# pathint/RankCompV3.jl

Hardware: AMD Instinct MI355X
Metric: gene-pair·sample comparisons/sec at 20k genes × 1k samples (higher is better)
Workload: dtype u16

## Files before the change

### rankcompv3.jl_amd/_ffi.py

```python
from __future__ import annotations

import ctypes
import os
import subprocess
from typing import NamedTuple

import numpy as np

_HERE = os.path.dirname(os.path.abspath(__file__))
LIB_PATH = os.environ.get("REO_LIB_PATH") or os.path.join(_HERE, "libreo_hip.so")
CSRC = os.path.join(_HERE, "csrc")

REO_OK, REO_EINVAL, REO_EHIP, REO_ECOMM, REO_ENOMEM = 0, -1, -2, -3, -4
NTIMINGS = 12
CALL_BINS = 8192

SYMBOLS = [
    "reo_version", "reo_last_error", "reo_create", "reo_destroy", "reo_trim_memory", "reo_set_shard", "reo_set_allreduce", "reo_set_allgather",
    "reo_create_multi", "reo_comm_unique_id", "reo_comm_init_rank",
    "reo_set_matrix_f64", "reo_set_matrix_i64", "reo_set_matrix_dev_f64", "reo_set_matrix_dev_i64",
    "reo_set_matrix_f32", "reo_set_matrix_i32", "reo_set_matrix_dev_f32", "reo_set_matrix_dev_i32",
    "reo_set_matrix_rm_f64", "reo_set_matrix_rm_i64", "reo_set_matrix_rm_f32", "reo_set_matrix_rm_i32",
    "reo_set_matrix_csc_f64", "reo_set_matrix_csc_i64", "reo_set_matrix_csc_f32", "reo_set_matrix_csc_i32",
    "reo_set_groups", "reo_compute_thresholds", "reo_set_thresholds", "reo_get_thresholds", "reo_threshold",
# ... 649 lines not shown
        pm = self._partner_mask(partner_mask)
        n_sel = np.zeros(g.size, dtype=np.int32)
        n_gt = np.zeros((g.size, max(self.S, 1)), dtype=np.int32)
        n_eq = np.zeros_like(n_gt) if ties else None
        self.sample_counts_raw(g, mask, pm, n_sel, n_gt, n_eq)
        return SampleCounts(g, n_sel, n_gt[:, : self.S], None if n_eq is None else n_eq[:, : self.S])

    def sample_scores(self, genes, partner_mask=None) -> SampleScores:
        return sample_scores_from(self.sample_counts(genes, "n13", partner_mask), self.sample_counts(genes, "n31", partner_mask))

    def sample_tests_raw(self, genes, partner_mask, n_above_ctrl, n_below_ctrl, rev_up, rev_down, tied, p_up, p_down) -> None:
        check(self._L.reo_sample_tests(self._h, *_genes(genes), _opt(partner_mask), _opt(n_above_ctrl), _opt(n_below_ctrl), _opt(rev_up),
                                       _opt(rev_down), _opt(tied), _opt(p_up), _opt(p_down)))

    def sample_tests(self, genes=None, partner_mask=None, counts=True) -> SampleTests:
        g = np.arange(self.G, dtype=np.int32) if genes is None else np.ascontiguousarray(genes, dtype=np.int32).reshape(-1)
        pm = self._partner_mask(partner_mask)
        shape = (g.size, max(self.S, 1))
        n_above, n_below = np.zeros(g.size, dtype=np.int32), np.zeros(g.size, dtype=np.int32)
        ints = [np.zeros(shape, dtype=np.int32) for _ in range(3)] if counts else [None] * 3
        p_up, p_down = np.ones(shape, dtype=np.float64), np.ones(shape, dtype=np.float64)
        self.sample_tests_raw(g, pm, n_above, n_below, ints[0], ints[1], ints[2], p_up, p_down)
        cut = lambda a: None if a is None else a[:, : self.S]
        return SampleTests(g, n_above, n_below, cut(ints[0]), cut(ints[1]), cut(ints[2]), cut(p_up), cut(p_down))

    def sample_calls_raw(self, genes, partner_mask, pval_deg: float, padj_deg: float, calls, cut, n_up, n_down) -> None:
        check(self._L.reo_sample_calls(self._h, *_genes(genes), _opt(partner_mask), float(pval_deg), float(padj_deg), _opt(calls), _opt(cut),
                                       _opt(n_up), _opt(n_down)))

    def sample_calls(self, pval_deg: float, padj_deg: float, genes=None, partner_mask=None) -> SampleCalls:
        g = np.arange(self.G, dtype=np.int32) if genes is None else np.ascontiguousarray(genes, dtype=np.int32).reshape(-1)
        pm = self._partner_mask(partner_mask)
        S = max(self.S, 1)
        calls = np.zeros((g.size, S), dtype=np.int8)
        cut, n_up, n_down = (np.zeros(S, dtype=np.int32) for _ in range(3))
        self.sample_calls_raw(g, pm, pval_deg, padj_deg, calls, cut, n_up, n_down)
        return SampleCalls(g, calls[:, : self.S], cut[: self.S], n_up[: self.S], n_down[: self.S])

    def pair_support_raw(self, genes, rowptr, partner, n_gt, n_eq, outcome) -> None:
        check(self._L.reo_pair_support(self._h, *_genes(genes), _opt(rowptr), _genes(partner)[0],
                                       _opt(n_gt), _opt(n_eq), _opt(outcome)))

    def pair_support(self, pairs, ties=True, outcomes=False) -> PairSupport:
        code = None
        if isinstance(pairs, PairList):
            genes, rowptr, partner, code = pairs
        else:
            genes, rowptr, partner = pairs
        g = np.ascontiguousarray(genes, dtype=np.int32).reshape(-1)
        rp = np.ascontiguousarray(rowptr, dtype=np.int64).reshape(-1)
        pa = np.ascontiguousarray(partner, dtype=np.int32).reshape(-1)
        if rp.size != g.size + 1:
            raise DimensionMismatch(REO_EINVAL, f"pair_support: rowptr has {rp.size} entries for {g.size} rows (one more is needed)")
        if rp.size and int(rp[-1]) != pa.size:
            raise DimensionMismatch(REO_EINVAL, f"pair_support: rowptr lists {int(rp[-1])} entries, partner has {pa.size}")
        if code is not None:
            code = np.asarray(code)
            if code.size != pa.size:
                raise DimensionMismatch(REO_EINVAL, f"pair_support: code has {code.size} entries, partner has {pa.size}")
        n, ng, S = pa.size, max(self.ngroups, 1), max(self.S, 1)
        n_gt = np.zeros((n, ng), dtype=np.int32)
        n_eq = np.zeros_like(n_gt) if ties else None
        outcome = np.zeros((n, S), dtype=np.uint8) if outcomes else None
        if g.size:
            self.pair_support_raw(g, rp, pa, n_gt, n_eq, outcome)
        sizes = np.bincount(np.asarray(self._group_id, dtype=np.int64), minlength=ng)[:ng].astype(np.int64)
        return PairSupport(g, rp, pa, code, n_gt, n_eq, None if outcome is None else outcome[:, : self.S], sizes)

    def mccullagh(self, cont) -> np.ndarray:
        cont = np.ascontiguousarray(cont, dtype=np.int32).reshape(-1, 9)
        out = np.zeros((cont.shape[0], 5), dtype=np.float64)
        check(self._L.reo_mccullagh(self._h, _ptr(cont), cont.shape[0], _ptr(out)))
        return out

    @staticmethod
    def _pseudobulk_args(cells, order, chunk_ptr):
        order = np.ascontiguousarray(order, dtype=np.int32)
        chunk_ptr = np.ascontiguousarray(chunk_ptr, dtype=np.int32)
        n_out = chunk_ptr.size - 1
        if hasattr(cells, "tocsc"):
            m = cells.tocsc()
            m.sort_indices()
            G, C = m.shape
            isint = np.issubdtype(m.dtype, np.integer)
            val = np.ascontiguousarray(m.data, dtype=np.int64 if isint else np.float64)
            colptr = np.ascontiguousarray(m.indptr, dtype=np.int64)
            rowidx = np.ascontiguousarray(m.indices, dtype=np.int32)
            args = (G, C, _ptr(colptr), _ptr(rowidx), _ptr(val), _ptr(order), order.size, _ptr(chunk_ptr), n_out)
            return "csc", "i64" if isint else "f64", args, G, (m, val, colptr, rowidx, order, chunk_ptr)
        X = np.asarray(cells)
        isint = np.issubdtype(X.dtype, np.integer)
        Xf = np.asfortranarray(X, dtype=np.int64 if isint else np.float64)
        G, C = Xf.shape
        args = (_ptr(Xf), G, C, G, _ptr(order), order.size, _ptr(chunk_ptr), n_out)
        return "dense", "i64" if isint else "f64", args, G, (Xf, order, chunk_ptr)

    def pseudobulk(self, cells, order, chunk_ptr) -> np.ndarray:
        form, ty, args, G, keep = self._pseudobulk_args(cells, order, chunk_ptr)
        out = np.zeros((G, args[-1]), dtype=np.int64 if ty == "i64" else np.float64, order="F")
        check(getattr(self._L, f"reo_pseudobulk_{form}_{ty}")(self._h, *args, _ptr(out)))
        return out

    def set_matrix_pseudobulk(self, cells, order, chunk_ptr) -> None:
        if is_device_sparse(cells) or is_device_tensor(cells):
            order = np.ascontiguousarray(order, dtype=np.int32)
            chunk_ptr = np.ascontiguousarray(chunk_ptr, dtype=np.int32)
            n_out = chunk_ptr.size - 1
            tail = (_ptr(order) if order.size else None, order.size, _ptr(chunk_ptr), n_out)
            if is_device_sparse(cells):
                ty, G, C, nnz, colptr, rowidx, val, bits, keep = device_csc_entry(cells)
                check(getattr(self._L, "reo_set_matrix_pseudobulk_csc_dev_" + ty)(self._h, G, C, nnz, _dptr(colptr), _dptr(rowidx), bits, _dptr(val), *tail))
            else:
                ptr, G, C, ld, ty, keep = device_matrix(cells)
                check(getattr(self._L, "reo_set_matrix_pseudobulk_dense_dev_" + ty)(self._h, ctypes.c_void_p(ptr), G, C, ld, *tail))
            self.G, self.S = G, n_out
            return
        form, ty, args, G, keep = self._pseudobulk_args(cells, order, chunk_ptr)
        check(getattr(self._L, f"reo_set_matrix_pseudobulk_{form}_{ty}")(self._h, *args))
        self.G, self.S = G, args[-1]

    def filter_matrix(self, min_profiles: int = 0, min_features: int = 0):
        info = self.info()
        pk = np.zeros(info["S"], dtype=np.uint8)
        gk = np.zeros(info["G"], dtype=np.uint8)
        sk, gkn = ctypes.c_int64(0), ctypes.c_int64(0)
        check(self._L.reo_filter_matrix(self._h, int(min_profiles), int(min_features), _ptr(pk) if pk.size else None, _ptr(gk) if gk.size else None,
                                        ctypes.byref(sk), ctypes.byref(gkn)))
        self.G, self.S = int(gkn.value), int(sk.value)
        return pk.astype(bool), gk.astype(bool)

    def get_matrix(self) -> np.ndarray:
        info = self.info()
        dt = {1: np.float64, 2: np.int64, 3: np.float32}.get(info["resident_dtype"])
        if dt is None:
            raise DimensionMismatch(REO_EINVAL, "no expression matrix set")
        out = np.zeros((info["G"], info["S"]), dtype=dt, order="F")
        check(self._L.reo_get_matrix(self._h, _ptr(out), out.nbytes))
        return out

    def set_profiling(self, on: bool) -> None:
        check(self._L.reo_set_profiling(self._h, 1 if on else 0))

    def reset_timings(self) -> None:
        check(self._L.reo_reset_timings(self._h))

    def timings(self) -> dict:
        ms = np.zeros(NTIMINGS, dtype=np.float64)
        check(self._L.reo_get_timings(self._h, _ptr(ms), NTIMINGS))
        return {"transform_ms": ms[0], "k1_ms": ms[1], "k2_ms": ms[2], "iter_ms": ms[3], "k3_ms": max(ms[3] - ms[2], 0.0), "k2_launches": int(ms[4]),
                "k1_launches": int(ms[5]), "exchange_ms": ms[6], "pseudobulk_ms": ms[7], "k2_full_ms": ms[8],
                "k2_full_launches": int(ms[9]), "k2_delta_ms": ms[10], "set_matrix_host_wall_ms": ms[11]}

    def info(self) -> dict:
        w = np.zeros(30, dtype=np.int64)
        check(self._L.reo_get_info(self._h, _ptr(w), 30))
        v = np.zeros(28, dtype=np.int64)
        v[:] = w[:28]
        return {"G": int(v[0]), "S": int(v[1]), "Gp": int(v[2]), "table_bytes": int(v[3]), "has_ties": int(v[4]),
                "tiles_owned": int(v[5]), "tiles_total": int(v[6]), "tile_i": int(v[7]), "chunk_j": int(v[8]),
                "chunks_per_panel": int(v[9]), "unit_h": int(v[10]), "sample_slots": int(v[11]),
                "shared_group_counts": int(v[12]), "group_count_bytes": int(v[13]), "transform_in_lds": int(v[14]), "xcc_local_histograms": int(v[15]),
                "cycle_period": int(v[16]), "cycle_found_at_pass": int(v[17]), "cycle_passes_skipped": int(v[18]), "upload_link_bytes": int(v[19]),
                "eager_range_launches": int(v[20]), "rowmajor_upload": int(v[21]),
                "csc_upload": int(v[22]), "csc_nnz": int(v[23]), "resident_dtype": int(v[24]),
                "k1_slot_order": int(v[25]), "k1_half_tiles_separated": int(v[26]), "csc_device": int(v[27]),
                "k1_unslot_form": int(w[28]), "contrast_treat": int(w[29])}
```

### rankcompv3.jl_amd/csrc/api.hip

```cpp
#include <execinfo.h>
#include <signal.h>
#include <unistd.h>

#include <ctime>
#include <algorithm>
#include <chrono>
#include <cmath>
#include <cstdarg>
#include <cstdio>
#include <cstdlib>
#include <cstring>

#include "reo_internal.h"
#include "contrast.h"
#include "upload_csc.h"

#include <mutex>
#include <unordered_map>

namespace reo {

static thread_local std::string g_err;
thread_local bool tl_release_synced = false;

// ... 157 lines not shown
void tic(reo_ctx *c, int slot)
{
    if (!c->profiling) return;
    StageTimer t;
    if (!c->pool.empty()) { t = c->pool.back(); c->pool.pop_back(); }
    else { (void)handle_event(&t.a, 1); (void)handle_event(&t.b, 1); }
    (void)hipEventRecord(t.a, c->stream);
    c->pending.emplace_back(slot, t);
    c->open.push_back(c->pending.size() - 1);
}

void toc(reo_ctx *c)
{
    if (!c->profiling || c->open.empty()) return;
    (void)hipEventRecord(c->pending[c->open.back()].second.b, c->stream);
    c->open.pop_back();
}

void collect_timings(reo_ctx *c)
{
    for (auto &pr : c->pending) {
        float ms = 0.f;
        (void)hipEventSynchronize(pr.second.b);
        if (hipEventElapsedTime(&ms, pr.second.a, pr.second.b) == hipSuccess) {
            c->t_ms[pr.first] += ms;
            if (pr.first == 2 && !c->k2_modes.empty()) {
                if (c->k2_seen < c->k2_modes.size()) {
                    if (c->k2_modes[c->k2_seen]) { c->t_ms[8] += ms; c->t_ms[9] += 1.0; }
                    else c->t_ms[10] += ms;
                }
                ++c->k2_seen;
            }
        }
        c->pool.push_back(pr.second);
    }
    c->pending.clear();
    c->open.clear();
    c->k2_modes.clear();
    c->k2_seen = 0;
}

static int32_t major_reo_lower_count(int32_t n, double thr)
{
    const long double ln2 = 0.693147180559945309417232121458L;
    long double logc = 0.0L, cdf_prev = 0.0L;
    int32_t first_above = -1;
    double pmin = 1.0;
    for (int x = 0; x <= n / 2; ++x) {
        if (x > 0) logc += std::log(static_cast<long double>(n - x + 1)) - std::log(static_cast<long double>(x));
        long double cdf = x >= n ? 1.0L : cdf_prev + std::exp(logc - static_cast<long double>(n) * ln2);
        if (cdf > 1.0L) cdf = 1.0L;
        const long double hi = 1.0L - cdf_prev;
        long double p = 2.0L * (cdf < hi ? cdf : hi);
        if (p > 1.0L) p = 1.0L;
        if (x == 0) {
            pmin = static_cast<double>(p);
            if (!(pmin < thr)) return n;
        }
        if (static_cast<double>(p) > thr) { first_above = x; break; }
        cdf_prev = cdf;
    }
    return first_above < 0 ? -1 : n - first_above + 1;
}

static hipError_t stream_wait(reo_ctx *c)
{
    if (!c->spin_wait) return hipStreamSynchronize(c->stream);
    for (unsigned spin = 0;; ++spin) {
        const hipError_t q = hipStreamQuery(c->stream);
        if (q != hipErrorNotReady) return q;
        if (spin > (1u << 22)) return hipStreamSynchronize(c->stream);
    }
}

static struct sigaction g_old_action[3];

static void segv_backtrace(int sig)
{
    static const char head[] = "libreo_hip: fatal signal, native backtrace of the faulting thread:\n";
    (void)!write(2, head, sizeof head - 1);
    void *frames[64];
    const int n = backtrace(frames, 64);
    backtrace_symbols_fd(frames, n, 2);
    sigaction(sig, &g_old_action[sig == SIGSEGV ? 0 : (sig == SIGBUS ? 1 : 2)], nullptr);
    raise(sig);
}

static void install_segv_backtrace()
{
    static bool done = false;
    if (done) return;
    done = true;
    void *warm[2];
    (void)backtrace(warm, 2);
    struct sigaction sa;
    memset(&sa, 0, sizeof sa);
    sa.sa_handler = segv_backtrace;
    sa.sa_flags = SA_NODEFER;
    sigaction(SIGSEGV, &sa, &g_old_action[0]);
    sigaction(SIGBUS, &sa, &g_old_action[1]);
    sigaction(SIGABRT, &sa, &g_old_action[2]);
}

static double wall_us()
{
    timespec ts;
    clock_gettime(CLOCK_MONOTONIC, &ts);
    return ts.tv_sec * 1e6 + ts.tv_nsec * 1e-3;
}

static void drop_ref_mask(reo_ctx *c, const char *why)
{
    c->ref_slot = -1;
    c->ref_gone = why;
}

int32_t wait_or_drop_table(reo_ctx *c)
{
    const hipError_t e = stream_wait(c);
    if (e == hipSuccess) return REO_OK;
    c->built_k = -1;
    c->table_complete = false;
    drop_ref_mask(c, "a kernel queued on this context failed and the class table was dropped");
    set_error("a kernel queued on this context failed: %s (the class table was dropped: call reo_build_pairs again)", hipGetErrorString(e));
    return REO_EHIP;
}

int32_t use(reo_ctx *c)
{
    if (!c) { set_error("null context"); return REO_EINVAL; }
    REO_HIP_CHECK(hipSetDevice(c->device));
    return REO_OK;
}

int32_t no_multi(reo_ctx *c, const char *what)
{
    if (!c) { set_error("null context"); return REO_EINVAL; }
    if (c->in_multi) {
        set_error("%s is not available on a reo_create_multi context (every device would need the matrix: use one process per GPU, each with its own context)", what);
        return REO_EINVAL;
    }
    return REO_OK;
}

static void invalidate(reo_ctx *c)
{
    drop_ref_mask(c, "the matrix or the groups changed after the last reo_identify_degs (reo_set_matrix_*, reo_filter_matrix, reo_set_groups): "
                     "the class table it ran on is gone");
    c->transformed = false;
    c->built_k = -1;
    c->built_treat = -1;
    c->gc_valid = false;
    c->eager_k1 = false;
    c->last_k1_slots = 0; c->k1_slot_items = nullptr; c->k1_slot_items_n = 0; c->k1_slot_gp = 0;
}

static size_t elem_bytes(int dtype) { return dtype >= 3 ? 4 : 8; }

static int32_t check_shape(int64_t G, int64_t S)
{
    if (G < 2 || G > kMaxGenes || S < 2 || S > (1 << 20)) {
        set_error("matrix is %lld x %lld; G must be in [2, %d] and S in [2, 1048576]", (long long)G, (long long)S, kMaxGenes);
        return REO_EINVAL;
    }
    return REO_OK;
}

static int32_t set_matrix(reo_ctx *c, const void *X, int64_t G, int64_t S, int64_t ld, int dtype, bool on_device, int layout = kLayoutColMajor)
{
    const bool rowmajor = layout == kLayoutRowMajor;
    int32_t rc = use(c);
    if (rc) return rc;
    if (dtype >= 3 && getenv("REO_TRANSFORM") && getenv("REO_TRANSFORM")[0] == 's') {
        set_error("REO_TRANSFORM=segmented: the segmented sort of the A/B build takes Float64 and Int64 matrices only, not Float32 / Int32");
        return REO_EINVAL;
    }
    if (!X) { set_error("matrix pointer is null"); return REO_EINVAL; }
    if ((rc = check_shape(G, S))) return rc;
    if (rowmajor && ld < S) { set_error("row pitch %lld < S = %lld (row-major: ld counts the elements from one gene's row to the next)", (long long)ld, (long long)S); return REO_EINVAL; }
    if (layout == kLayoutColMajor && ld < G) { set_error("leading dimension %lld < G = %lld", (long long)ld, (long long)G); return REO_EINVAL; }
    invalidate(c);
    c->rowmajor_upload = 0;
    c->csc_upload = 0; c->csc_nnz = 0; c->csc_device = 0;
    const bool host_i32 = dtype == 4 && !on_device;
    const size_t resident = static_cast<size_t>(G) * S * (dtype == 3 ? 4 : 8);
    c->G = G; c->S = S; c->dtype = dtype == 4 ? 2 : dtype;
    if (on_device && dtype == 4) {
        if ((rc = c->dX_owned.ensure(resident))) return rc;
        c->dX = c->dX_owned.p; c->ld = G;
        if ((rc = widen_device_i32(c, X, ld, G, S, c->dX_owned.p))) { invalidate(c); c->dtype = 0; return rc; }
        if (hipStreamSynchronize(c->stream) != hipSuccess) { set_error("widening the Int32 matrix failed"); invalidate(c); c->dtype = 0; return REO_EHIP; }
    } else if (on_device) {
        c->dX = X; c->ld = ld;
        c->dX_owned.release();
    } else {
        if ((rc = c->dX_owned.ensure(resident))) return rc;
        c->dX = c->dX_owned.p; c->ld = G;
        const bool lds_ranking = G <= 65535 && !(getenv("REO_TRANSFORM") && getenv("REO_TRANSFORM")[0] == 's');
        if (c->eager_mode > 0 && lds_ranking && static_cast<int64_t>(c->group_id.size()) == S && !c->in_multi) {
            const bool k1 = c->eager_mode > 1 && c->ngroups == 2 && c->thr_set && c->world <= 1 && !c->comm && !c->ag && !c->ar && c->k1_wave &&
                            S <= 65535 && !c->k1_stamps;
            c->Gp = static_cast<int>((c->G + kGenePad - 1) / kGenePad) * kGenePad;
            c->Wp = c->Gp / 32;
            if ((rc = c->table.ensure(static_cast<size_t>(c->G) * kPlanes * c->Wp))) return rc;
            const double w0 = wall_us();
            struct DrainUp {
                reo_ctx *c;
                ~DrainUp() { if (c->up) (void)hipStreamSynchronize(c->up); if (c->rk) (void)hipStreamSynchronize(c->rk); }
            } drain_up{c};
            DrainOnExit drain(c);
            rc = eager_upload(c, X, ld, k1, host_i32, layout);
            if (rc) { invalidate(c); return rc; }
            c->rowmajor_upload = rowmajor ? 1 : 0;
            c->csc_upload = layout == kLayoutCsc ? 1 : 0;
            drain.dismiss();
            c->t_ms[11] += (wall_us() - w0) * 1e-3;
            if (c->eager_k1) { c->built_k = 0; c->table_complete = true; }
            return REO_OK;
        }
        struct DrainUp2 {
            reo_ctx *c;
            ~DrainUp2() { if (c->up) (void)hipStreamSynchronize(c->up); }
        } drain_up{c};
        DrainOnExit drain(c);
        const double w0 = wall_us();
        if ((rc = upload_columns(c, X, ld, G, S, c->dX_owned.p, dtype, layout))) { invalidate(c); return rc; }
        c->rowmajor_upload = rowmajor ? 1 : 0;
        c->csc_upload = layout == kLayoutCsc ? 1 : 0;
        drain.dismiss();
        c->t_ms[11] += (wall_us() - w0) * 1e-3;
    }
    return REO_OK;
}

int32_t ensure_transform(reo_ctx *c)
{
    if (c->dtype == 0) { set_error("no expression matrix set"); return REO_EINVAL; }
    if (c->group_id.empty()) { set_error("no groups set"); return REO_EINVAL; }
    if (static_cast<int64_t>(c->group_id.size()) != c->S) {
        set_error("'data' and 'group' do not have compatible sizes (%lld columns, %zu group labels)",
                  (long long)c->S, c->group_id.size());
        return REO_EINVAL;
    }
    if (c->transformed) return REO_OK;
    c->Gp = static_cast<int>((c->G + kGenePad - 1) / kGenePad) * kGenePad;
    c->Wp = c->Gp / 32;
    c->table_prezeroed = false;
    int32_t rc = c->table.ensure(static_cast<size_t>(c->G) * kPlanes * c->Wp);
    if (rc) return rc;
    return run_transform(c);
}

static int32_t ensure_iter_buffers(reo_ctx *c)
{
    int32_t rc;
    const size_t G = c->G;
    for (int t = 0; t < 2; ++t) {
        if ((rc = c->refbits[t].ensure(c->Wp))) return rc;
        if ((rc = c->refbytes[t].ensure(c->Gp))) return rc;
    }
    if ((rc = c->raw.ensure(G * kRaw)) ||
        (rc = c->delta_list.ensure(2 * static_cast<size_t>(c->Gp))) || (rc = c->cont.ensure(G * 9)) || (rc = c->result.ensure(G * 15)) ||
        (rc = c->sorted_d.ensure((G + 63) / 64 * 64 + (G + 63) / 64)) || (rc = c->sorted_p.ensure(G)) || (rc = c->rank_s.ensure(G)) ||
        (rc = c->rank_a.ensure(G)) || (rc = c->scal.ensure(8)) || (rc = c->blockmin.ensure(std::max<size_t>(64, (G + 1023) / 1024))) ||
        (rc = c->state.ensure(1)) ||
        (rc = c->chunk_v.ensure(((G + kSortChunk - 1) / kSortChunk) * (kSortChunk + kSortChunk / 32))) ||
        (rc = c->chunk_i.ensure(((G + kSortChunk - 1) / kSortChunk) * kSortChunk)) || (rc = c->part.ensure(3 * (std::max<size_t>(65536, (G + kSortChunk - 1) / kSortChunk * kSortChunk) / 16 + 8))) ||
        (rc = c->cand.ensure(2 * 1024)) || (rc = c->gridbar.ensure(4)) || (rc = c->hist.ensure(3 * kHistParts * ((G + 32767) / 32768 * 32768))) || (rc = c->olist.ensure(2 * kOneStride)) || (rc = c->mrank.ensure(c->Gp)) || (rc = c->lstate.ensure(1)) || (rc = c->clist.ensure(2 * kListStride)) || (rc = c->scal.ensure(64)))
        return rc;
    if (!c->host_state) REO_HIP_CHECK(pool_alloc(reinterpret_cast<void **>(&c->host_state), sizeof(IterState), true));
    return REO_OK;
}

static int32_t upload_ref(reo_ctx *c, const uint8_t *ref, int slot, int32_t *nref)
{
    int32_t n = 0;
    for (int64_t i = 0; i < c->G; ++i) n += ref[i] != 0;
    *nref = n;
    REO_HIP_CHECK(hipMemsetAsync(c->refbytes[slot].p, 0, c->Gp, c->stream));
    REO_HIP_CHECK(hipMemcpyAsync(c->refbytes[slot].p, ref, c->G, hipMemcpyHostToDevice, c->stream));
    return launch_pack_ref(c, c->refbytes[slot].p, c->refbits[slot].p);
}

static int32_t init_state(reo_ctx *c, int32_t nref)
{
    IterState st;
    memset(&st, 0, sizeof st);
    st.nref = nref;
    st.nref_prev = nref;
    st.delta_cnt[0] = st.delta_cnt[1] = 0x7FFFFFFF;
    st.need_full = 1;
    st.raw_pass = -1;
    st.kstar = -1;
    *c->host_state = st;
    REO_HIP_CHECK(hipMemcpyAsync(c->state.p, c->host_state, sizeof st, hipMemcpyHostToDevice, c->stream));
    return REO_OK;
}

static int32_t exchange_table(reo_ctx *c)
{
    if (c->x_pipelined) {
        c->table_complete = true;
        return REO_OK;
    }
    c->table_complete = c->world <= 1;
    if (c->world <= 1 && !c->comm) return REO_OK;
    int32_t rc;
    if (c->comm || c->ag) {
        const int64_t bytes = exchange_unit_words(c) * exchange_units_per_rank(c) * static_cast<int64_t>(sizeof(uint32_t));
        if ((rc = c->xsend.ensure(static_cast<size_t>(bytes / 4))) || (rc = c->xrecv.ensure(static_cast<size_t>(bytes / 4) * c->world))) return rc;
        tic(c, 6);
        if ((rc = launch_pack_units(c))) return rc;
        if (c->comm) {
            if ((rc = comm_allgather(c, c->xsend.p, c->xrecv.p, bytes)) < 0) return rc;
        } else {
            rc = c->ag(c->xsend.p, c->xrecv.p, bytes, c->stream, c->ag_user);
            if (rc) { set_error("all-gather hook failed with %d", rc); return REO_ECOMM; }
        }
        if ((rc = launch_expand_units(c))) return rc;
        toc(c);
    } else {
        if (!c->ar) return REO_OK;
        const int64_t count = static_cast<int64_t>(c->G) * kPlanes * c->Wp;
        tic(c, 6);
        rc = c->ar(c->table.p, count, c->stream, c->ar_user);
        toc(c);
        if (rc) { set_error("all-reduce hook failed with %d", rc); return REO_ECOMM; }
    }
    c->table_complete = true;
    return REO_OK;
}

static int32_t pass_fault(reo_ctx *c)
{
    const int32_t f = c->host_state ? c->host_state->fault : 0;
    if (!f) return REO_OK;
    if (f == kFaultTallies) {
        set_error("the iteration passes met tallies that no class table can produce (a gene pair in two states at once): the table in "
                  "this context is not what reo_build_pairs makes -- an exchange hook delivered wrong words and the scan of its "
                  "table was switched off (REO_CHECK_HOOK_TABLE=0)");
        c->built_k = -1;
        c->table_complete = false;
    } else {
        set_error("the persistent iteration kernel gave up at a grid barrier (a workgroup did not arrive within its bound); "
                  "REO_LIGHT=1 runs the same passes as separate launches");
    }
    return REO_EHIP;
}

int32_t upload_slot2col(reo_ctx *c, const std::vector<int32_t> &map)
{
    if (map == c->sc_slot2col_host && c->sc_slot2col.p == c->sc_slot2col_uploaded) return REO_OK;
    c->sc_slot2col_host = map;
    c->sc_slot2col_uploaded = nullptr;
    REO_HIP_CHECK(hipMemcpyAsync(c->sc_slot2col.p, c->sc_slot2col_host.data(), map.size() * sizeof(int32_t), hipMemcpyHostToDevice, c->stream));
    c->sc_slot2col_uploaded = c->sc_slot2col.p;
    return REO_OK;
}

int32_t need_complete_table(reo_ctx *c)
{
    if (c->built_k < 0) { set_error("no class table: call reo_build_pairs first"); return REO_EINVAL; }
    if (!c->table_complete) {
        set_error("shard %d of %d holds only its own part of the class table: attach a communicator (reo_comm_init_rank) or an "
                  "exchange hook (reo_set_allgather, reo_set_allreduce) before reo_build_pairs", c->rank, c->world);
        return REO_ECOMM;
    }
    return REO_OK;
}

}

using namespace reo;

extern "C" {

int32_t reo_version(void) { return 1100; }

int32_t reo_trim_memory(void)
{
    std::vector<Block> all;
    {
        Pool &P = pool();
        std::lock_guard<std::mutex> lk(P.mu);
        all.swap(P.free_blocks);
        P.cached = 0;
    }
    int dev = 0;
    const bool have_dev = hipGetDevice(&dev) == hipSuccess;
    for (const Block &b : all) {
        if (!b.pinned) (void)hipSetDevice(b.device);
        raw_free(b.p, b.pinned);
    }
    {
        Handles &H = handles();
        std::lock_guard<std::mutex> lk(H.mu);
        for (int k = 0; k < 2; ++k) {
            for (auto &st : H.streams[k]) { (void)hipSetDevice(st.first); (void)hipStreamDestroy(st.second); }
            for (auto &ev : H.events[k]) { (void)hipSetDevice(ev.first); (void)hipEventDestroy(ev.second); }
            H.streams[k].clear(); H.events[k].clear();
        }
    }
    if (have_dev) (void)hipSetDevice(dev);
    return REO_OK;
}

const char *reo_last_error(void) { return g_err.c_str(); }

int32_t reo_create(reo_ctx **out, int32_t device, uint64_t seed)
{
    if (!out) { set_error("out is null"); return REO_EINVAL; }
    *out = nullptr;
    if (getenv("REO_DEBUG_SEGV")) install_segv_backtrace();
    int ndev = 0;
    if (hipGetDeviceCount(&ndev) != hipSuccess || ndev == 0) {
        set_error("no HIP device visible: libreo_hip has no CPU fallback");
        return REO_EHIP;
    }
    if (device < 0) REO_HIP_CHECK(hipGetDevice(&device));
    if (device >= ndev) { set_error("device %d out of range (%d visible)", device, ndev); return REO_EINVAL; }
    hipDeviceProp_t prop;
    REO_HIP_CHECK(hipGetDeviceProperties(&prop, device));
    if (strncmp(prop.gcnArchName, "gfx950", 6) != 0) {
        set_error("device %d is %s; this library carries gfx950 (MI355X) code objects only", device, prop.gcnArchName);
        return REO_EHIP;
    }
    REO_HIP_CHECK(hipSetDevice(device));
    reo_ctx *c = new (std::nothrow) reo_ctx();
    if (!c) { set_error("out of host memory"); return REO_ENOMEM; }
    c->device = device;
    c->seed = seed;
    if (const char *e = getenv("REO_K1_WAVE")) c->k1_wave = (e[0] != '0');
    if (const char *e = getenv("REO_K1_HALF")) c->k1_half = (e[0] != '0');
    if (const char *e = getenv("REO_K1_SLOTS")) c->k1_slots = (e[0] != '0');
    if (const char *e = getenv("REO_K1_QUEUE")) c->k1_queue = (e[0] != '0');
    if (const char *e = getenv("REO_K1_UNSLOT")) { const int v = atoi(e); c->k1_unslot = (v == 8 || v == 4) ? v : (e[0] == '0' ? 0 : -1); }
    if (const char *e = getenv("REO_K1_WORKERS")) c->k1_workers = std::max(1, atoi(e));
    if (const char *e = getenv("REO_K1_ORDER")) c->k1_order = std::max(0, std::min(2, atoi(e)));
    {
        int n = 0;
        if (hipDeviceGetAttribute(&n, hipDeviceAttributeMultiprocessorCount, c->device) == hipSuccess && n > 0) c->n_cus = n;
    }
    if (const char *e = getenv("REO_SPIN_WAIT")) c->spin_wait = (e[0] != '0');
    if (const char *e = getenv("REO_CHECK_HOOK_TABLE")) c->check_hook_table = (e[0] != '0');
    if (const char *e = getenv("REO_SHARE_GROUP_COUNTS")) c->share_counts = (e[0] != '0');
    if (const char *e = getenv("REO_LIGHT_BAND")) c->light_band = std::max(0, atoi(e));
    if (const char *e = getenv("REO_HIST_BELOW")) c->hist_below = std::max(0, atoi(e));
    if (const char *e = getenv("REO_CYCLE")) c->cycle_watch = atoi(e) != 0;
    if (const char *e = getenv("REO_LIGHT")) c->light_mode = e[0] == '0' ? 0 : (e[0] == '2' ? 2 : (e[0] == '3' ? 3 : 1));
    c->light_window = light_window(); c->light_min_g = light_min_genes();
    if (const char *e = getenv("REO_LIGHT_WINDOW")) c->light_window = std::max(1, std::min(31, atoi(e)));
    if (const char *e = getenv("REO_LIGHT_MIN_G")) c->light_min_g = std::max(64, atoi(e));
    if (const char *e = getenv("REO_STATE_MIRROR")) c->state_mirror_wanted = (e[0] != '0');
    if (const char *e = getenv("REO_EXCHANGE_WAVES")) c->x_waves = std::max(1, std::min(8, atoi(e)));
    if (const char *e = getenv("REO_EAGER_UPLOAD")) c->eager_mode = std::max(0, std::min(2, atoi(e)));
    if (const char *e = getenv("REO_EAGER_CHUNK")) c->eager_chunk = std::max(1, atoi(e));
    if (const char *e = getenv("REO_EAGER_GATE")) c->eager_gate = atoi(e) != 0;
    if (const char *e = getenv("REO_EAGER_RANGES")) c->eager_ranges = std::max(1, std::min(6, atoi(e)));
    if (const char *e = getenv("REO_UPLOAD_THREADS")) c->upload_threads = std::max(0, std::min(64, atoi(e)));
    c->debug_passes = getenv("REO_DEBUG_PASSES") != nullptr;
    c->debug_stamps = getenv("REO_DEBUG_STAMPS") != nullptr;
    c->k1_stamps = getenv("REO_K1_STAMPS") != nullptr;
    hipError_t e = handle_stream(&c->stream, 0);
    if (e != hipSuccess) { delete c; set_error("hipStreamCreate failed: %s", hipGetErrorString(e)); return REO_EHIP; }
    int ok = 0;
    const char *xe = getenv("REO_XCC_LOCAL");
    if (!(xe && xe[0] == '0')) {
        const int32_t rc = xcc_selftest(c, &ok);
        if (rc) { reo_destroy(c); return rc; }
    }
    c->xcc_local = ok;
    *out = c;
    return REO_OK;
}

void reo_destroy(reo_ctx *c)
{
    if (!c) return;
    for (reo_ctx *p : c->peers) reo_destroy(p);
    c->peers.clear();
    (void)hipSetDevice(c->device);
    for (int q = 0; q < 2; ++q) if (c->k1s[q]) (void)hipStreamSynchronize(c->k1s[q]);
    if (c->xs) (void)hipStreamSynchronize(c->xs);
    if (c->up) (void)hipStreamSynchronize(c->up);
    if (c->rk) (void)hipStreamSynchronize(c->rk);
    (void)hipStreamSynchronize(c->stream);
    comm_release(c);
    collect_timings(c);
    tl_release_synced = true;
    for (auto &t : c->pool) { release_event(t.a, 1); release_event(t.b, 1); }
    c->dX_owned.release(); c->pos.release(); c->lo.release(); c->hi.release(); c->goff_dev.release();
    c->table.release();
    c->t_kin.release(); c->t_kout.release(); c->t_vin.release(); c->t_vout.release(); c->t_temp.release();
    c->t_order.release(); c->t_flags.release(); c->t_slots.release(); c->unit_map.release();
    for (auto &il : c->k1_wave_items) il.buf.release();
    for (int q = 0; q < 2; ++q) { release_stream(c->k1s[q], 0); release_event(c->ev_k1_join[q], 0); }
    release_stream(c->xs, 0);
    release_stream(c->up, 0);
    release_stream(c->rk, 1);
    for (auto &e : c->ev_rk) release_event(e, 0);
    for (auto &e : c->ev_up) release_event(e, 0);
    c->e_lists.release();
    for (int q = 0; q < 3; ++q) {
        if (c->stage_h[q]) pool_free(c->stage_h[q], c->stage_cap, true);
        c->stage_d[q].release();
        release_event(c->ev_stage[q], 0);
        release_event(c->ev_widen[q], 0);
    }
    release_event(c->ev_fork, 0);
    release_event(c->ev_x, 0);
    for (auto &e : c->ev_k1) release_event(e, 0);
    c->t_pos16.release(); c->t_lo16.release(); c->t_hi16.release(); c->gcounts.release();
    c->k1_slot_part.release(); c->k1_slot_maps.release(); c->pos_s.release(); c->lo_s.release(); c->k1_queue_ctr.release();
    c->t_pos32.release(); c->t_lo32.release(); c->t_hi32.release(); c->t_vin32.release(); c->t_vout32.release();
    for (int t = 0; t < 2; ++t) { c->refbits[t].release(); c->refbytes[t].release(); }
    c->raw.release(); c->delta_list.release(); c->cont.release(); c->result.release(); c->sorted_d.release(); c->sorted_p.release();
    c->rank_s.release(); c->rank_a.release(); c->scal.release(); c->blockmin.release();
    c->state.release(); c->trace.release(); c->modes.release(); c->cand.release(); c->hist.release(); c->mrank.release(); c->lstate.release(); c->clist.release(); c->olist.release(); c->units_all.release(); c->xsend.release(); c->xrecv.release(); c->check_flag.release(); c->gridbar.release(); c->chunk_v.release(); c->chunk_i.release(); c->part.release();
    if (c->host_state) pool_free(c->host_state, sizeof(IterState), true);
    if (c->host_flags) pool_free(c->host_flags, 8 * sizeof(int32_t), true);
    release_event(c->ev_flags, 0);
    if (c->host_ref) pool_free(c->host_ref, c->host_ref_cap, true);
    release_stream(c->stream, 0);
    delete c;
    tl_release_synced = false;
}

int32_t reo_set_shard(reo_ctx *c, int32_t rank, int32_t world)
{
    if (!c) { set_error("null context"); return REO_EINVAL; }
    if (world < 1 || rank < 0 || rank >= world) { set_error("bad shard %d of %d", rank, world); return REO_EINVAL; }
    if (!c->peers.empty()) { set_error("a multi-GPU context (reo_create_multi) shards by itself"); return REO_EINVAL; }
    c->rank = rank; c->world = world;
    c->built_k = -1;
    drop_ref_mask(c, "reo_set_shard dropped the class table that the last reo_identify_degs ran on");
    c->eager_k1 = false;
    c->gc_valid = false;
    c->table_complete = false;
    return REO_OK;
}

int32_t reo_set_allreduce(reo_ctx *c, reo_allreduce_fn fn, void *user)
{
    if (!c) { set_error("null context"); return REO_EINVAL; }
    c->ar = fn; c->ar_user = user;
    return REO_OK;
}

int32_t reo_set_allgather(reo_ctx *c, reo_allgather_fn fn, void *user)
{
    if (!c) { set_error("null context"); return REO_EINVAL; }
    c->ag = fn; c->ag_user = user;
    return REO_OK;
}

static int32_t set_matrix_all(reo_ctx *c, const void *X, int64_t G, int64_t S, int64_t ld, int dtype, bool on_device, int layout = kLayoutColMajor)
{
    int32_t rc = set_matrix(c, X, G, S, ld, dtype, on_device, layout);
    for (size_t d = 0; d < (c ? c->peers.size() : 0) && !rc; ++d) {
        reo_ctx *p = c->peers[d];
        if (!on_device) { rc = set_matrix(p, X, G, S, ld, dtype, false, layout); continue; }
        const void *src = dtype == 4 ? c->dX : X;
        const int64_t sld = dtype == 4 ? G : ld;
        const size_t eb = dtype == 4 ? 8 : elem_bytes(dtype);
        if ((rc = use(p)) || (rc = p->dX_owned.ensure(static_cast<size_t>(G) * S * eb))) break;
        if (hipMemcpy2DAsync(p->dX_owned.p, static_cast<size_t>(G) * eb, src, static_cast<size_t>(sld) * eb, static_cast<size_t>(G) * eb, static_cast<size_t>(S),
                             hipMemcpyDefault, p->stream) != hipSuccess) {
            set_error("peer copy of the matrix to device %d failed", p->device); rc = REO_EHIP;
        }
        if (!rc && hipStreamSynchronize(p->stream) != hipSuccess) { set_error("peer copy failed"); rc = REO_EHIP; }
        if (!rc) { invalidate(p); p->G = G; p->S = S; p->dtype = dtype == 4 ? 2 : dtype; p->dX = p->dX_owned.p; p->ld = G; }
    }
    if (c && !c->peers.empty()) (void)hipSetDevice(c->device);
    return rc;
}

int32_t reo_set_matrix_f64(reo_ctx *c, const double *X, int64_t G, int64_t S, int64_t ld) { return set_matrix_all(c, X, G, S, ld, 1, false); }
int32_t reo_set_matrix_i64(reo_ctx *c, const int64_t *X, int64_t G, int64_t S, int64_t ld) { return set_matrix_all(c, X, G, S, ld, 2, false); }
int32_t reo_set_matrix_dev_f64(reo_ctx *c, const void *dX, int64_t G, int64_t S, int64_t ld) { return set_matrix_all(c, dX, G, S, ld, 1, true); }
int32_t reo_set_matrix_dev_i64(reo_ctx *c, const void *dX, int64_t G, int64_t S, int64_t ld) { return set_matrix_all(c, dX, G, S, ld, 2, true); }
int32_t reo_set_matrix_f32(reo_ctx *c, const float *X, int64_t G, int64_t S, int64_t ld) { return set_matrix_all(c, X, G, S, ld, 3, false); }
int32_t reo_set_matrix_i32(reo_ctx *c, const int32_t *X, int64_t G, int64_t S, int64_t ld) { return set_matrix_all(c, X, G, S, ld, 4, false); }
int32_t reo_set_matrix_dev_f32(reo_ctx *c, const void *dX, int64_t G, int64_t S, int64_t ld) { return set_matrix_all(c, dX, G, S, ld, 3, true); }
int32_t reo_set_matrix_dev_i32(reo_ctx *c, const void *dX, int64_t G, int64_t S, int64_t ld) { return set_matrix_all(c, dX, G, S, ld, 4, true); }
int32_t reo_set_matrix_rm_f64(reo_ctx *c, const double *X, int64_t G, int64_t S, int64_t ld) { return set_matrix_all(c, X, G, S, ld, 1, false, kLayoutRowMajor); }
int32_t reo_set_matrix_rm_i64(reo_ctx *c, const int64_t *X, int64_t G, int64_t S, int64_t ld) { return set_matrix_all(c, X, G, S, ld, 2, false, kLayoutRowMajor); }
int32_t reo_set_matrix_rm_f32(reo_ctx *c, const float *X, int64_t G, int64_t S, int64_t ld) { return set_matrix_all(c, X, G, S, ld, 3, false, kLayoutRowMajor); }
int32_t reo_set_matrix_rm_i32(reo_ctx *c, const int32_t *X, int64_t G, int64_t S, int64_t ld) { return set_matrix_all(c, X, G, S, ld, 4, false, kLayoutRowMajor); }

// ... 461 lines not shown
                for (int q = 1; q <= nlight; ++q)
                    if (hs.slot[q].pad0[0] || q <= 3)
                        fprintf(stderr, "  launch %d: why %d (1 window, 2 se left the bracket, 4 the histogram's cut left the band, 8 a list overflowed, 16 too many listed, 32 cut below the band), "
                                "cut of the m_lo histogram %d, listed %d, surely inside %d, cut %d (band around %d), eta %.3g, se %.10g\n", q, hs.slot[q].pad0[0], hs.slot[q].pad0[1],
                                hs.slot[q].pad0[2], hs.slot[q].pad0[3], hs.slot[q].pad0[4], hs.slot[q - 1].rec.kstar, hs.slot[q - 1].eta, hs.slot[q].se_base);
        }
        if (c->debug_passes)
            fprintf(stderr, "batch: %d sorting + %d light launches, passes %d -> %d, need_full %d, done %d, last_full %d, changed genes in front of the next pass %d\n", nfull, nlight,
                    passes, c->host_state->passes, c->host_state->need_full, c->host_state->done, c->host_state->last_full,
                    c->host_state->delta_cnt[c->host_state->passes & 1]);
        if ((rc = pass_fault(c))) return rc;
        idle_any = c->host_state->passes == passes ? idle_any + 1 : 0;
        if (idle_any >= 4) {
            set_error("the iteration made no progress in four batches of launches (passes %d, need_full %d): loop control fault", passes, c->host_state->need_full);
            return REO_EHIP;
        }
        if (nlight > 0) idle_light = c->host_state->passes == passes ? idle_light + 1 : 0;
        if (idle_light >= 2 && !small) {
            small = true;
            c->it_no_light = true;
        }
        if (c->host_state->passes < passes || c->host_state->passes > n_iter) {
            set_error("the iteration's pass counter reads %d after %d of %d passes: loop control fault", c->host_state->passes, passes, n_iter);
            return REO_EHIP;
        }
        passes = c->host_state->passes;
        seen_need_full = c->host_state->need_full;
        if (c->host_state->done || passes >= n_iter) break;
        if (c->host_state->cyc_period > 0) {
            const int p = c->host_state->cyc_period, P = (p & 1) ? 2 * p : p;
            const int skip = (n_iter - passes - 1) / P * P;
            if ((rc = launch_cycle_skip(c, skip, p))) return rc;
            c->it_cycle_period = p; c->it_cycle_at = passes; c->it_cycle_skipped = skip;
            if (c->debug_passes) fprintf(stderr, "cycle: the reference set in front of pass %d equals that of pass %d; %d passes skipped\n", passes, passes - p, skip);
            passes += skip;
        }
    }
    if (passes > 0 && !c->host_state->last_full) {
        tic(c, 3);
        if ((rc = launch_full_pass(c, true))) return rc;
        toc(c);
    }
    if (trace && passes > 0)
        REO_HIP_CHECK(hipMemcpyAsync(trace, c->trace.p, sizeof(int32_t) * 2 * passes, hipMemcpyDeviceToHost, c->stream));
    const int nk2 = std::min<int>(c->k2_idx, static_cast<int>(c->modes.n));
    if (c->profiling && nk2 > 0) {
        c->k2_modes.assign(c->k2_idx, 0);
        REO_HIP_CHECK(hipMemcpyAsync(c->k2_modes.data(), c->modes.p, sizeof(int32_t) * nk2, hipMemcpyDeviceToHost, c->stream));
    }
    if (c->debug_stamps) {
        unsigned long long st[24];
        REO_HIP_CHECK(hipMemcpy(st, c->scal.p + 32, sizeof st, hipMemcpyDeviceToHost));
        if (light_form == 3) {
            fprintf(stderr, "stamps kl_one (inputs back, se, cut, lists + mask step, changed rows, delta1, sums + windows, end):");
            for (int k = 0; k <= 7; ++k) fprintf(stderr, " %lld", (long long)(st[k] - st[8]));
        } else if (light_form == 2) {
            fprintf(stderr, "stamps kl_persist, one pass (phase 1, barrier, phase 2, barrier, loads asked, cut, mask step):");
            for (int k = 1; k <= 7; ++k) fprintf(stderr, " %lld", (long long)(st[k] - st[0]));
        } else {
            fprintf(stderr, "stamps kl_head (inputs back, cut, mask step, changed rows, delta1, window flags, block sums, end):");
            for (int k = 0; k <= 7; ++k) fprintf(stderr, " %lld", (long long)(st[k] - st[8]));
            fprintf(stderr, "\nstamps kl_rank (inputs back, selection + se, p + BH rank, end):");
            for (int k = 20; k <= 23; ++k) fprintf(stderr, " %lld", (long long)(st[k] - st[19]));
        }
        fprintf(stderr, "  (x 10 ns)\n");
    }
    if (iters_run) *iters_run = passes;
    const double w_copy = c->debug_passes ? wall_us() : 0.0;
    REO_HIP_CHECK(hipMemcpyAsync(result, c->result.p, sizeof(double) * 15 * G, hipMemcpyDeviceToHost, c->stream));
    const double w_copied = c->debug_passes ? wall_us() : 0.0;
    if ((rc = wait_or_drop_table(c))) return rc;
    drain.dismiss();
    if (c->debug_passes) fprintf(stderr, "  result copy: enqueued in %.0f us, waited %.0f us\n", w_copied - w_copy, wall_us() - w_copied);
    collect_timings(c);
    if ((rc = pass_fault(c))) return rc;
    if (passes > 0) c->ref_slot = (passes - 1) & 1;
    else drop_ref_mask(c, "the last reo_identify_degs was called with n_iter <= 0: no pass ran, no tallies were counted");
    return REO_OK;
}

int32_t reo_get_ref_mask(reo_ctx *c, uint8_t *ref_mask, int32_t *nref)
{
    int32_t rc = use(c);
    if (rc) return rc;
    if (!ref_mask) { set_error("reo_get_ref_mask: ref_mask must not be null"); return REO_EINVAL; }
    if (c->ref_slot < 0 || c->built_k < 0) {
        set_error("reo_get_ref_mask: no reference set to deliver: %s", c->ref_slot < 0 ? c->ref_gone : "the class table was dropped");
        return REO_EINVAL;
    }
    DrainOnExit drain(c);
    REO_HIP_CHECK(hipMemcpyAsync(ref_mask, c->refbytes[c->ref_slot].p, static_cast<size_t>(c->G), hipMemcpyDeviceToHost, c->stream));
    REO_HIP_CHECK(hipStreamSynchronize(c->stream));
    drain.dismiss();
    int32_t n = 0;
    for (int64_t i = 0; i < c->G; ++i) { ref_mask[i] = ref_mask[i] != 0; n += ref_mask[i]; }
    if (nref) *nref = n;
    return REO_OK;
}

int32_t reo_mccullagh(reo_ctx *c, const int32_t *cont, int64_t n, double *out)
{
    int32_t rc = use(c);
    if (rc) return rc;
    if (!cont || !out || n < 1) { set_error("bad argument"); return REO_EINVAL; }
    DevBuf<int32_t> dc;
    DevBuf<double> dout;
    if ((rc = dc.ensure(n * 9)) || (rc = dout.ensure(n * 5))) return rc;
    DrainOnExit drain(c);
    hipError_t e = hipMemcpyAsync(dc.p, cont, sizeof(int32_t) * 9 * n, hipMemcpyHostToDevice, c->stream);
    if (e == hipSuccess) {
        rc = launch_mccullagh(c, dc.p, n, dout.p);
        if (!rc) {
            e = hipMemcpyAsync(out, dout.p, sizeof(double) * 5 * n, hipMemcpyDeviceToHost, c->stream);
            if (e == hipSuccess) e = hipStreamSynchronize(c->stream);
        }
    }
    if (e != hipSuccess) { set_error("HIP failure: %s", hipGetErrorString(e)); rc = REO_EHIP; }
    dc.release(); dout.release();
    return rc;
}

int32_t reo_set_profiling(reo_ctx *c, int32_t on)
{
    if (!c) { set_error("null context"); return REO_EINVAL; }
    c->profiling = on != 0;
    for (reo_ctx *p : c->peers) p->profiling = c->profiling;
    return REO_OK;
}

int32_t reo_reset_timings(reo_ctx *c)
{
    if (!c) { set_error("null context"); return REO_EINVAL; }
    collect_timings(c);
    for (double &v : c->t_ms) v = 0.0;
    return REO_OK;
}

int32_t reo_get_timings(reo_ctx *c, double *ms, int32_t n)
{
    if (!c || !ms) { set_error("null argument"); return REO_EINVAL; }
    collect_timings(c);
    for (int i = 0; i < n && i < REO_NTIMINGS; ++i) ms[i] = c->t_ms[i];
    return REO_OK;
}

int32_t reo_get_info(reo_ctx *c, int64_t *info, int32_t n)
{
    if (!c || !info) { set_error("null argument"); return REO_EINVAL; }
    int64_t separated = 0;
    if (n > 26 && c->last_k1_slots) {
        int32_t rc = use(c);
        if (rc || (rc = launch_slot_separated(c, &separated))) return rc;
    }
    const int64_t v[30] = {c->G, c->S, c->Gp, static_cast<int64_t>(c->table.n * sizeof(uint32_t)), c->has_ties,
                           c->tiles_owned, c->tiles_total, kTileI, c->k1_cj, c->k1_q, kUnitH,
                           c->goff32.empty() ? 0 : c->goff32.back(), c->last_k1_shared,
                           static_cast<int64_t>(c->gcounts.n * sizeof(uint16_t)), c->transform_in_lds, c->xcc_local,
                           c->it_cycle_period, c->it_cycle_at, c->it_cycle_skipped, c->narrowed_bytes, c->eager_range_launches, c->rowmajor_upload,
                           c->csc_upload, c->csc_nnz, c->dtype, c->last_k1_slots, separated, c->csc_device,
                           c->last_k1_slots ? c->last_k1_unslot : 0, c->built_k >= 0 ? c->built_treat : -1};
    for (int i = 0; i < n && i < 30; ++i) info[i] = v[i];
    return REO_OK;
}

}
```

### rankcompv3.jl_amd/csrc/k1_slots.h

```cpp
#pragma once

#include <cstddef>
#include <cstdint>

#if defined(__HIPCC__) || defined(__CUDACC__)
#define REO_SLOTS_HD __host__ __device__ inline
#else
#define REO_SLOTS_HD inline
#endif

namespace reo {

constexpr int kSlotTile = 32;
constexpr int kSlotChunk = 256;
constexpr uint32_t kSlotNoMin = 0xFFFFu, kSlotNoMax = 0u;

REO_SLOTS_HD uint32_t slot_pack(uint32_t mn, uint32_t mx) { return mn | mx << 16; }
REO_SLOTS_HD uint32_t slot_min(uint32_t w) { return w & 0xFFFFu; }
REO_SLOTS_HD uint32_t slot_max(uint32_t w) { return w >> 16; }
REO_SLOTS_HD uint32_t slot_join(uint32_t a, uint32_t b)
{
    const uint32_t mn = slot_min(a) < slot_min(b) ? slot_min(a) : slot_min(b), mx = slot_max(a) > slot_max(b) ? slot_max(a) : slot_max(b);
    return slot_pack(mn, mx);
}

REO_SLOTS_HD uint32_t slot_key(uint32_t side0, uint32_t side1) { return slot_min(side0) + slot_max(side0) + slot_min(side1) + slot_max(side1); }

REO_SLOTS_HD uint64_t slot_order_key(uint32_t key, uint32_t gene) { return static_cast<uint64_t>(key) << 32 | gene; }

REO_SLOTS_HD int slot_separated(uint32_t tile_rng, uint32_t chunk_rng)
{
    if (slot_max(chunk_rng) < slot_min(tile_rng)) return 1;
    if (slot_max(tile_rng) < slot_min(chunk_rng)) return -1;
    return 0;
}

REO_SLOTS_HD int slot_item_tile(uint32_t item) { return static_cast<int>(item & 0x3FFFu); }
REO_SLOTS_HD int slot_item_chunk(uint32_t item) { return static_cast<int>((item >> 16) & 0x7FFFu); }
REO_SLOTS_HD int slot_item_side(uint32_t item) { return static_cast<int>(item >> 31); }
REO_SLOTS_HD int slot_item_halves(uint32_t item) { return (item & 0x8000u) ? 1 : 2; }


inline void slot_rank(const uint32_t *key, int G, uint32_t *g2s)
{
    for (int g = 0; g < G; ++g) {
        uint32_t n = 0;
        for (int h = 0; h < G; ++h) n += slot_order_key(key[h], static_cast<uint32_t>(h)) < slot_order_key(key[g], static_cast<uint32_t>(g)) ? 1u : 0u;
        g2s[g] = n;
    }
}

inline void slot_invert(const uint32_t *g2s_G, int G, int Gp, uint32_t *g2s, uint32_t *s2g)
{
    for (int g = 0; g < G; ++g) { g2s[g] = g2s_G[g]; s2g[g2s_G[g]] = static_cast<uint32_t>(g); }
    for (int g = G; g < Gp; ++g) g2s[g] = s2g[g] = static_cast<uint32_t>(g);
}

inline void slot_unpermute_row(const uint32_t *in, uint32_t *out, int W, const uint32_t *g2s, int G)
{
    for (int w = 0; w < W; ++w) out[w] = 0;
    for (int j = 0; j < G; ++j) {
        const uint32_t k = g2s[j];
        out[j >> 5] |= ((in[k >> 5] >> (k & 31)) & 1u) << (j & 31);
    }
}

constexpr int kUnslotWide = 8, kUnslotNarrow = 4;
constexpr size_t kUnslotLdsLimit = 160 * 1024;
constexpr int kUnslotThreadsMax = 1024;

REO_SLOTS_HD int unslot_bit(int row, int plane) { return 4 * row + plane; }

REO_SLOTS_HD uint32_t unslot_lds_index(int form, uint32_t k)
{
    const uint32_t w = k >> 5, b = k & 31u;
    return form == kUnslotWide ? 33u * w + b : 2u * (17u * w + (b & 15u)) + (b >> 4);
}

REO_SLOTS_HD size_t unslot_lds_bytes(int form, int Gp) { return static_cast<size_t>(Gp / 32) * (form == kUnslotWide ? 33u * 4u : 17u * 4u); }

REO_SLOTS_HD int unslot_form(int Gp)
{
    if (3 * unslot_lds_bytes(kUnslotNarrow, Gp) <= kUnslotLdsLimit) return kUnslotNarrow;
    return unslot_lds_bytes(kUnslotWide, Gp) <= kUnslotLdsLimit ? kUnslotWide : kUnslotNarrow;
}

REO_SLOTS_HD int unslot_threads(int Wp)
{
    const int trips = (Wp + kUnslotThreadsMax - 1) / kUnslotThreadsMax;
    return ((Wp + trips - 1) / trips + 63) / 64 * 64;
}

#if defined(__clang__)
#define REO_SLOTS_UNROLL _Pragma("unroll")
#else
#define REO_SLOTS_UNROLL
#endif

template <int N>
REO_SLOTS_HD void unslot_transpose(uint32_t (&w)[N])
{
    static_assert(N == 32 || N == 16, "4 R words");
    uint32_t m = N == 32 ? 0x0000FFFFu : 0x00FF00FFu;
    REO_SLOTS_UNROLL
    for (int j = N / 2; j != 0; j >>= 1, m ^= (m << j)) {
        REO_SLOTS_UNROLL
        for (int k = 0; k < N; k = (k + j + 1) & ~j) {
            const uint32_t t = ((w[k] >> j) ^ w[k + j]) & m;
            w[k] ^= t << j;
            w[k + j] ^= t;
        }
    }
}

template <int R>
REO_SLOTS_HD void unslot_in_word(uint32_t (&m)[4 * R], int w, uint32_t *T)
{
    unslot_transpose<4 * R>(m);
    if (R == kUnslotWide) {
        REO_SLOTS_UNROLL
        for (int b = 0; b < 4 * R; ++b) T[unslot_lds_index(R, 32u * w + b)] = m[b];
    } else {
        REO_SLOTS_UNROLL
        for (int i = 0; i < 4 * R; ++i) T[unslot_lds_index(R, 32u * w + i) >> 1] = m[i];
    }
}

template <int R>
REO_SLOTS_HD void unslot_out_word(uint32_t (&u)[4 * R], const uint32_t (&ks)[32], int wo, const uint32_t *T, int G, int Gp)
{
    if (R == kUnslotWide) {
        REO_SLOTS_UNROLL
        for (int c = 0; c < 32; ++c) {
            const uint32_t k = ks[c] < static_cast<uint32_t>(Gp) ? ks[c] : static_cast<uint32_t>(Gp - 1);
            u[c % (4 * R)] = T[unslot_lds_index(R, k)];
        }
    } else {
        const uint16_t *T16 = reinterpret_cast<const uint16_t *>(T);
        REO_SLOTS_UNROLL
        for (int c = 0; c < 32; ++c) {
            const uint32_t k = ks[c] < static_cast<uint32_t>(Gp) ? ks[c] : static_cast<uint32_t>(Gp - 1);
            const uint32_t e = T16[unslot_lds_index(R, k)];
            if (c < 16) u[c % (4 * R)] = e;
            else u[c % (4 * R)] |= e << 16;
        }
    }
    unslot_transpose<4 * R>(u);
    const int left = G - 32 * wo;
    const uint32_t valid = left >= 32 ? 0xFFFFFFFFu : (left <= 0 ? 0u : (1u << left) - 1u);
    REO_SLOTS_UNROLL
    for (int q = 0; q < 4 * R; ++q) u[q] &= valid;
}

template <int R>
inline void unslot_group_model(uint32_t *table, int r0, int n_rows, int G, int Wp, const uint32_t *g2s, uint32_t *T)
{
    const int nr = n_rows - r0 < R ? n_rows - r0 : R;
    if (nr <= 0) return;
    uint32_t *rows = table + static_cast<size_t>(r0) * 4 * Wp;
    for (int w = 0; w < Wp; ++w) {
        uint32_t m[4 * R];
        for (int q = 0; q < 4 * R; ++q) m[q] = q < 4 * nr ? rows[static_cast<size_t>(q) * Wp + w] : 0u;
        unslot_in_word<R>(m, w, T);
    }
    for (int wo = 0; wo < Wp; ++wo) {
        uint32_t u[4 * R], ks[32];
        for (int c = 0; c < 32; ++c) ks[c] = g2s[32 * wo + c];
        unslot_out_word<R>(u, ks, wo, T, G, 32 * Wp);
        for (int q = 0; q < 4 * nr; ++q) rows[static_cast<size_t>(q) * Wp + wo] = u[q];
    }
}

inline void slot_permute_row(const uint32_t *in, uint32_t *out, int W, const uint32_t *s2g, int G)
{
    for (int w = 0; w < W; ++w) out[w] = 0;
    for (int k = 0; k < G; ++k) {
        const uint32_t j = s2g[k];
        out[k >> 5] |= ((in[j >> 5] >> (j & 31)) & 1u) << (k & 31);
    }
}

}
```

### rankcompv3.jl_amd/csrc/kernels.hip

```cpp
#include <algorithm>
#include <chrono>
#include <cstddef>
#include <cstdio>
#include <cstdlib>
#include <cstring>
#include <mutex>
#include <type_traits>

#include "reo_internal.h"
#include "k1_items.h"
#include "k1_slots.h"
#include "k1_queue.h"
#include "contrast.h"

namespace reo {

namespace {

__device__ __forceinline__ uint64_t mix64(uint64_t z)
{
    z += 0x9E3779B97F4A7C15ULL;
    z = (z ^ (z >> 30)) * 0xBF58476D1CE4E5B9ULL;
    z = (z ^ (z >> 27)) * 0x94D049BB133111EBULL;
    return z ^ (z >> 31);
// ... 79 lines not shown
    for (int r = 0; r < RJ; ++r)
#pragma unroll
        for (int h = 0; h < RI / 2; ++h) { gt[r][h] = 0; if (TIES) ge[r][h] = 0; }
    if (bb >= be) return;
    uint4 sl[kPerThread], sh[TIES ? kPerThread : 1];
    auto stage_load = [&](int b0) {
#pragma unroll
        for (int e = 0; e < kPerThread; ++e) {
            const int idx = threadIdx.x + 256 * e;
            const int b = min(b0 + idx / (RI * 4), be - 1);
            const size_t o = (static_cast<size_t>(b) * Gp + i0) * 4 + idx % (RI * 4);
            sl[e] = AL[o];
            if (TIES) sh[e] = AH[o];
        }
    };
    auto stage_store = [&](int buf) {
#pragma unroll
        for (int e = 0; e < kPerThread; ++e) {
            sm_lo[buf * kStageQ + threadIdx.x + 256 * e] = sl[e];
            if (TIES) sm_hi[buf * kStageQ + threadIdx.x + 256 * e] = sh[e];
        }
    };
    stage_load(bb);
    __syncthreads();
    stage_store(0);
    __syncthreads();
    int buf = 0;
    for (int b0 = bb; b0 < be; b0 += kStageB) {
        const bool more = b0 + kStageB < be;
        if (more) stage_load(b0 + kStageB);
        const int nb = idle ? 0 : min(kStageB, be - b0);
        for (int s = 0; s < nb; ++s) {
            Planes16 p[RJ];
#pragma unroll
            for (int r = 0; r < RJ; ++r)
#pragma unroll
                for (int q = 0; q < NQ; ++q) p[r].set(q, P[(static_cast<size_t>(b0 + s) * 4 + q) * Gp + jl + 64 * r]);
            const uint4 *al = sm_lo + buf * kStageQ + s * RI * 4;
            const uint4 *ah = sm_hi + buf * kStageQ + s * RI * 4;
#pragma clang loop unroll(full)
            for (int i = 0; i < RI; ++i) {
                Planes16 a, c;
#pragma unroll
                for (int q = 0; q < 4; ++q) {
                    if (q < 3 && 4 * q + 1 > NB - 1) continue;
                    a.set(q, al[i * 4 + q]);
                    if (TIES) c.set(q, ah[i * 4 + q]);
                }
                uint32_t l[4];
                if (TIES) {
                    chains_first(l, p[0].w[0], p[1].w[0], p[0].w[0], p[1].w[0], a.w[a_word(0)], a.w[a_word(0)], c.w[a_word(0)], c.w[a_word(0)]);
#pragma unroll
                    for (int k = 1; k < NB; ++k)
                        chains_next(l, p[0].w[k], p[1].w[k], p[0].w[k], p[1].w[k], a.w[a_word(k)], a.w[a_word(k)], c.w[a_word(k)], c.w[a_word(k)]);
                } else {
                    chains_first(l, p[0].w[0], p[1].w[0], p[RJ - 2].w[0], p[RJ - 1].w[0], a.w[a_word(0)], a.w[a_word(0)], a.w[a_word(0)], a.w[a_word(0)]);
#pragma unroll
                    for (int k = 1; k < NB; ++k)
                        chains_next(l, p[0].w[k], p[1].w[k], p[RJ - 2].w[k], p[RJ - 1].w[k], a.w[a_word(k)], a.w[a_word(k)], a.w[a_word(k)], a.w[a_word(k)]);
                }
#pragma unroll
                for (int ch = 0; ch < 4; ++ch) {
                    uint32_t &dst = TIES ? (ch < 2 ? gt[ch][i >> 1] : ge[ch - 2][i >> 1]) : gt[ch % RJ][i >> 1];
                    if (i & 1) dst += static_cast<uint32_t>(__builtin_popcount(l[ch])) << 16;
                    else dst += static_cast<uint32_t>(__builtin_popcount(l[ch]));
                }
            }
        }
        if (more) stage_store(buf ^ 1);
        __syncthreads();
        buf ^= 1;
    }
}

struct K1Args {
    const uint4 *P;
    const uint4 *AL;
    const uint4 *AH;
    uint32_t *table;
    const uint32_t *unit_map;
    int G, Gp, Wp;
    int cb, ce, tb, te;
    int gc, gt;
    int nc, nt;
    int m1, m2;
    uint64_t seed;
    int n_units, Q;
    const int32_t *goff;
    int ngroups;
    const uint32_t *items;
    unsigned long long *stamps;
    const int32_t *gate;
    uint32_t *park;
    int32_t *park_ge;
    int park_mode;
    const uint32_t *s2g;
    const uint32_t *trng, *crng;
    uint32_t *queue;
    uint32_t n_items;
};
constexpr size_t kParkSlot = 2 * 64 * 64;

template <int RJ>
__device__ __forceinline__ bool wave_idle(int jw, int i0, int G)
{
    return jw >= G || ((jw + 64 * RJ - 1) >> 6) < (i0 >> 6);
}

__device__ __forceinline__ void shift_in(uint32_t &w, unsigned long long mask)
{
    unsigned long long carry_out;
    asm("v_addc_co_u32 %0, %1, %0, %0, %2" : "+v"(w), "=s"(carry_out) : "s"(mask));
}

__device__ __forceinline__ void write_lane(uint32_t &v, uint32_t x, int l)
{
    asm("v_writelane_b32 %0, %1, %2" : "+v"(v) : "s"(x), "i"(l));
}

template <int RI, int NEAR, typename F>
__device__ __forceinline__ void emit_rows(bool near, int d, unsigned long long lanes_ok, int hi_thr, int lo_thr, uint32_t &wL, uint32_t &wH,
                                          uint32_t &fLlo, uint32_t &fLhi, uint32_t &fHlo, uint32_t &fHhi, F val)
{
#pragma unroll
    for (int ii = RI - 1; ii >= 0; --ii) {
        const int n = val(ii);
        const unsigned long long ok = (NEAR == 1 || (NEAR == 2 && near)) ? (__ballot(d > ii) & lanes_ok) : lanes_ok;
        const unsigned long long mH = __ballot(n >= hi_thr) & ok;
        const unsigned long long mL = __ballot(n <= lo_thr) & ok & ~mH;
        shift_in(wH, mH);
        shift_in(wL, mL);
        write_lane(fHlo, static_cast<uint32_t>(mH), ii);
        write_lane(fHhi, static_cast<uint32_t>(mH >> 32), ii);
        write_lane(fLlo, static_cast<uint32_t>(mL), ii);
        write_lane(fLhi, static_cast<uint32_t>(mL >> 32), ii);
    }
}

template <int RI, bool SPLIT, bool SLOTS = false, typename F>
__device__ __forceinline__ void emit_gene(const K1Args &a, int i0, int j, int bi, int lane, int pl, int hi_thr, int lo_thr, F val)
{
    const int bj = __builtin_amdgcn_readfirstlane(j >> 6);
    if ((bj << 6) >= a.Gp || bj < bi) return;
    const int d = j - i0;
    const bool near = (bj << 6) - i0 < RI;
    const unsigned long long lanes_ok = __ballot(j < a.G);
    uint32_t wL = 0, wH = 0;
    uint32_t fLlo = 0, fLhi = 0, fHlo = 0, fHhi = 0;
    if (!SPLIT) emit_rows<RI, 2>(near, d, lanes_ok, hi_thr, lo_thr, wL, wH, fLlo, fLhi, fHlo, fHhi, val);
    else if (near) emit_rows<RI, 1>(near, d, lanes_ok, hi_thr, lo_thr, wL, wH, fLlo, fLhi, fHlo, fHhi, val);
    else emit_rows<RI, 0>(near, d, lanes_ok, hi_thr, lo_thr, wL, wH, fLlo, fLhi, fHlo, fHhi, val);
    const bool diag = (bj == bi);
    if (lane < RI && i0 + lane < a.G) {
        const size_t gi = SLOTS ? a.s2g[i0 + lane] : static_cast<size_t>(i0 + lane);
        uint32_t *row = a.table + (gi * kPlanes + pl) * a.Wp + 2 * bj;
        if (!diag) {
            *reinterpret_cast<uint2 *>(row) = uint2{fLlo, fLhi};
            *reinterpret_cast<uint2 *>(row + a.Wp) = uint2{fHlo, fHhi};
        } else {
            if (fLlo) atomicOr(row, fLlo);
            if (fLhi) atomicOr(row + 1, fLhi);
            if (fHlo) atomicOr(row + a.Wp, fHlo);
            if (fHhi) atomicOr(row + a.Wp + 1, fHhi);
        }
    }
    if (j < a.G) {
        const size_t gj = SLOTS ? a.s2g[j] : static_cast<size_t>(j);
        uint32_t *row = a.table + (gj * kPlanes + pl) * a.Wp + (i0 >> 5);
        if (RI == 16) {
            const int half = (i0 >> 4) & 1;
            if (!diag) {
                reinterpret_cast<uint16_t *>(row)[half] = static_cast<uint16_t>(wH);
                reinterpret_cast<uint16_t *>(row + a.Wp)[half] = static_cast<uint16_t>(wL);
            } else {
                if (wH) atomicOr(row, wH << (16 * half));
                if (wL) atomicOr(row + a.Wp, wL << (16 * half));
            }
        } else if (!diag) {
            row[0] = wH; row[a.Wp] = wL;
        } else {
            if (wH) atomicOr(row, wH);
            if (wL) atomicOr(row + a.Wp, wL);
        }
    }
}

template <int RI>
__device__ __forceinline__ void emit_constant(const K1Args &a, int i0, int jl, int side, int n)
{
    static_assert(kSlotChunk % 64 == 0 && kSlotChunk >= 64 && kSlotTile <= 64, "a tile's 64-gene block lies inside its chunk (slot_separated)");
    const int lane = threadIdx.x, bi = i0 >> 6;
    const int hi_thr = side ? a.m2 : a.m1, lo_thr = (side ? a.nt : a.nc) - hi_thr;
    int fwd = side ? 2 : 0, mir = fwd;
    if (n >= hi_thr) ++fwd;
    else if (n <= lo_thr) ++mir;
    else return;
    const bool row_ok = lane < RI && i0 + lane < a.G;
    uint32_t *frow = a.table + (static_cast<size_t>(row_ok ? a.s2g[i0 + lane] : 0u) * kPlanes + fwd) * a.Wp;
#pragma unroll
    for (int r = 0; r < kRJ; ++r) {
        const int j = jl + 64 * r;
        const int bj = __builtin_amdgcn_readfirstlane(j >> 6);
        if ((bj << 6) >= a.Gp || bj <= bi) continue;
        const unsigned long long lanes_ok = __ballot(j < a.G);
        if (!lanes_ok) continue;
        if (row_ok) *reinterpret_cast<uint2 *>(frow + 2 * bj) = uint2{static_cast<uint32_t>(lanes_ok), static_cast<uint32_t>(lanes_ok >> 32)};
        if (j < a.G) {
            uint32_t *row = a.table + (static_cast<size_t>(a.s2g[j]) * kPlanes + mir) * a.Wp + (i0 >> 5);
            if (RI == 16) reinterpret_cast<uint16_t *>(row)[(i0 >> 4) & 1] = 0xFFFFu;
            else *row = 0xFFFFFFFFu;
        }
    }
}

template <int RI, int RJ, typename F>
__device__ __forceinline__ void emit_side(const K1Args &a, int i0, int jl, int bi, int lane, int pl, int hi_thr, int lo_thr, F val)
{
#pragma unroll
    for (int r = 0; r < RJ; ++r)
        emit_gene<RI, false>(a, i0, jl + 64 * r, bi, lane, pl, hi_thr, lo_thr, [&](int ii) { return val(r, ii); });
}

template <int RI, int RJ>
__device__ __forceinline__ bool tile_of_block(const K1Args &a, int &i0, int &jl)
{
    const int slot = blockIdx.x & 7, q = blockIdx.x >> 3;
    const int bu = kUnitH * a.Q;
    const int u = (q / bu) * 8 + slot;
    if (u >= a.n_units) return false;
    const uint32_t um = a.unit_map[u];
    const int wq = q % bu;
    const int it = static_cast<int>(um & 0xFFFFu) * kUnitH + wq / a.Q;
    const int jc = static_cast<int>(um >> 16) * a.Q + wq % a.Q;
    i0 = it * RI;
    constexpr int CJ = kTileJ * RJ;
    if (i0 >= a.Gp || jc * CJ >= a.Gp) return false;
    jl = jc * CJ + (threadIdx.x >> 6) * (64 * RJ) + (threadIdx.x & 63);
    return ((jc * CJ + CJ - 1) >> 6) >= (i0 >> 6);
}

template <int RJ, bool TIES>
__device__ __forceinline__ int count_with_coins(const uint32_t (&gt)[RJ][kTileI / 2], const uint32_t (&ge)[TIES ? RJ : 1][kTileI / 2],
                                                uint64_t seed, int i0, int jl, int r, int ii, int g)
{
    int nre = static_cast<int>(unpack16(gt[r], ii));
    if (TIES) {
        const uint32_t neq = unpack16(ge[r], ii) - static_cast<uint32_t>(nre);
        if (neq) nre += tie_wins(seed, i0 + ii, jl + 64 * r, g, neq);
    }
    return nre;
}

template <int NB, bool TIES, bool MULTI>
__global__ __launch_bounds__(256, MULTI ? 2 : 3) void k1_pairs(K1Args a)
{
    constexpr int RI = kTileI, RJ = TIES ? kRJTies : kRJ;
    int i0, jl;
    if (!tile_of_block<RI, RJ>(a, i0, jl)) return;
    const int lane = threadIdx.x & 63, bi = i0 >> 6;
    __shared__ uint4 sm_lo[2 * kStageB * RI * 4];
    __shared__ uint4 sm_hi[TIES ? 2 * kStageB * RI * 4 : 1];
    const bool idle = wave_idle<RJ>(jl & ~63, i0, a.G);
    uint32_t gt[RJ][RI / 2], ge[TIES ? RJ : 1][RI / 2];

    count_pass<RJ, NB, TIES>(a.P, a.AL, a.AH, a.Gp, i0, jl, a.cb, a.ce, gt, ge, sm_lo, sm_hi, idle);
    emit_side<RI, RJ>(a, i0, jl, bi, lane, 0, a.m1, a.nc - a.m1,
                      [&](int r, int ii) { return count_with_coins<RJ, TIES>(gt, ge, a.seed, i0, jl, r, ii, a.gc); });
    if (!MULTI) {
        count_pass<RJ, NB, TIES>(a.P, a.AL, a.AH, a.Gp, i0, jl, a.tb, a.te, gt, ge, sm_lo, sm_hi, idle);
        emit_side<RI, RJ>(a, i0, jl, bi, lane, 2, a.m2, a.nt - a.m2,
                          [&](int r, int ii) { return count_with_coins<RJ, TIES>(gt, ge, a.seed, i0, jl, r, ii, a.gt); });
    } else {
        uint32_t tot[RJ][RI / 2];
#pragma unroll
        for (int r = 0; r < RJ; ++r)
#pragma unroll
            for (int h = 0; h < RI / 2; ++h) tot[r][h] = 0;
        for (int g = 0; g < a.ngroups; ++g) {
            if (g == a.gc) continue;
            count_pass<RJ, NB, TIES>(a.P, a.AL, a.AH, a.Gp, i0, jl, a.goff[g], a.goff[g + 1], gt, ge, sm_lo, sm_hi, idle);
#pragma unroll
            for (int r = 0; r < RJ; ++r)
#pragma unroll
                for (int h = 0; h < RI / 2; ++h) {
                    if (TIES) {
                        const uint32_t n0 = count_with_coins<RJ, TIES>(gt, ge, a.seed, i0, jl, r, 2 * h, g);
                        const uint32_t n1 = count_with_coins<RJ, TIES>(gt, ge, a.seed, i0, jl, r, 2 * h + 1, g);
                        tot[r][h] += n0 | (n1 << 16);
                    } else tot[r][h] += gt[r][h];
                }
        }
        emit_side<RI, RJ>(a, i0, jl, bi, lane, 2, a.m2, a.nt - a.m2, [&](int r, int ii) { return static_cast<int>(unpack16(tot[r], ii)); });
    }
}


#include "k1_loop_gen.inc"

template <int NB>
__device__ __forceinline__ void k1_loop(u32x16 &c0, u32x16 &c1, u32x16 &c2, u32x16 &c3, const void *pb, uint32_t ps, const void *ab,
                                        uint32_t as, uint32_t nblk, uint32_t poff, uint32_t aoff, uint32_t lds)
{
    if (NB == 12) k1_loop_nb12_free(c0, c1, c2, c3, pb, ps, ab, ab, as, nblk, poff, aoff, lds);
    else if (NB == 15) k1_loop_nb15_free(c0, c1, c2, c3, pb, ps, ab, ab, as, nblk, poff, aoff, lds);
    else if (NB == 16) k1_loop_nb16_free(c0, c1, c2, c3, pb, ps, ab, ab, as, nblk, poff, aoff, lds);
    else if (NB == 17) k1_loop_nb17_free(c0, c1, c2, c3, pb, ps, ab, ab, as, nblk, poff, aoff, lds);
    else k1_loop_nb18_free(c0, c1, c2, c3, pb, ps, ab, ab, as, nblk, poff, aoff, lds);
}

template <int NB>
__device__ __forceinline__ void k1_loop(u32x8 &c0, u32x8 &c1, u32x8 &c2, u32x8 &c3, const void *pb, uint32_t ps, const void *ab,
                                        uint32_t as, uint32_t nblk, uint32_t poff, uint32_t aoff, uint32_t lds)
{
    if (NB == 12) k1_loop_nb12_free_h(c0, c1, c2, c3, pb, ps, ab, ab, as, nblk, poff, aoff, lds);
    else if (NB == 15) k1_loop_nb15_free_h(c0, c1, c2, c3, pb, ps, ab, ab, as, nblk, poff, aoff, lds);
    else if (NB == 16) k1_loop_nb16_free_h(c0, c1, c2, c3, pb, ps, ab, ab, as, nblk, poff, aoff, lds);
    else if (NB == 17) k1_loop_nb17_free_h(c0, c1, c2, c3, pb, ps, ab, ab, as, nblk, poff, aoff, lds);
    else k1_loop_nb18_free_h(c0, c1, c2, c3, pb, ps, ab, ab, as, nblk, poff, aoff, lds);
}

template <int NB, bool TIES, int RI, bool SLOTS = false>
__device__ __forceinline__ void k1w_item(const K1Args &a, uint4 *ring, uint32_t idx, int i0, int jw, int side, unsigned long long t_begin)
{
    constexpr int RJ = kRJ, NE = TIES ? 2 : 1;
    constexpr bool BIG = NB > 16;
    constexpr int LQ = BIG ? 5 : 4, ROWB = BIG ? 128 : 64;
    typedef typename std::conditional<RI == 32, u32x16, u32x8>::type Counts;
    const int lane = threadIdx.x, jl = jw + lane, bi = i0 >> 6;
    const int bb = side ? a.tb : a.cb, be = side ? a.te : a.ce;
    Counts gt0, gt1, gt2, gt3;
    constexpr bool PARK_REGS = NB > 16;
    uint32_t park[(TIES && !PARK_REGS) ? RJ * (RI / 2) : 1];
    Counts ge0 = 0, ge1 = 0, ge2 = 0, ge3 = 0;
    unsigned long long t_loop = 0, t_emit = 0;
    if (a.stamps) t_loop = __builtin_amdgcn_s_memrealtime();
    int sep = 0;
    if constexpr (SLOTS) sep = __builtin_amdgcn_readfirstlane(slot_separated(a.trng[side * (a.Gp >> 5) + (i0 >> 5)], a.crng[side * (a.Gp >> 8) + (jw >> 8)]));
    if (SLOTS && sep) {
        emit_constant<RI>(a, i0, jl, side, sep > 0 ? (side ? a.nt : a.nc) : 0);
    } else if (be > bb) {
        const char *pb = reinterpret_cast<const char *>(a.P) + static_cast<size_t>(bb) * LQ * a.Gp * 16;
        const size_t aoff = (static_cast<size_t>(bb) * a.Gp + i0) * ROWB;
        const uint32_t lds = static_cast<uint32_t>(reinterpret_cast<uintptr_t>(ring));
#pragma clang loop unroll(disable)
        for (int e = 0; e < NE; ++e) {
            const char *ab = reinterpret_cast<const char *>(e ? a.AL : (TIES ? a.AH : a.AL)) + aoff;
            k1_loop<NB>(gt0, gt1, gt2, gt3, pb, static_cast<uint32_t>(a.Gp) * 16u, ab, static_cast<uint32_t>(a.Gp) * static_cast<uint32_t>(ROWB),
                        static_cast<uint32_t>(be - bb), static_cast<uint32_t>(jl) * 16u, static_cast<uint32_t>(lane) * 16u, lds);
            if (TIES && e == 0) {
                if constexpr (PARK_REGS) { ge0 = gt0; ge1 = gt1; ge2 = gt2; ge3 = gt3; }
                else {
                    constexpr int W = (TIES && !PARK_REGS) ? RI / 2 : 0;
#pragma unroll
                    for (int h = 0; h < W; ++h) { park[h] = gt0[h]; park[W + h] = gt1[h]; park[2 * W + h] = gt2[h]; park[3 * W + h] = gt3[h]; }
                }
            }
        }
    } else {
        gt0 = 0; gt1 = 0; gt2 = 0; gt3 = 0;
#pragma unroll
        for (int h = 0; h < ((TIES && !PARK_REGS) ? RJ * (RI / 2) : 1); ++h) park[h] = 0;
    }
    if (a.stamps) t_emit = __builtin_amdgcn_s_memrealtime();
    if (!SLOTS && a.park_mode) {
        constexpr int W4 = RI / 8;
        uint4 *slot = reinterpret_cast<uint4 *>(a.park + static_cast<size_t>(idx) * kParkSlot) + lane;
        auto add4 = [&](Counts &v, const uint4 *p) {
#pragma unroll
            for (int q = 0; q < W4; ++q) { const uint4 w = p[q * 64]; v[4 * q] += w.x; v[4 * q + 1] += w.y; v[4 * q + 2] += w.z; v[4 * q + 3] += w.w; }
        };
        auto put4 = [&](const Counts &v, uint4 *p) {
#pragma unroll
            for (int q = 0; q < W4; ++q) p[q * 64] = uint4{v[4 * q], v[4 * q + 1], v[4 * q + 2], v[4 * q + 3]};
        };
        if (a.park_mode & 1) {
            const uint4 *ge_from = slot + ((TIES && __builtin_amdgcn_readfirstlane(a.park_ge[idx])) ? 4 * W4 * 64 : 0);
            if constexpr (TIES && PARK_REGS) { add4(ge0, ge_from); add4(ge1, ge_from + W4 * 64); add4(ge2, ge_from + 2 * W4 * 64); add4(ge3, ge_from + 3 * W4 * 64); }
            else if constexpr (TIES) {
#pragma clang loop unroll(disable)
                for (int cq = 0; cq < 4 * W4; ++cq) { const uint4 w = ge_from[cq * 64]; park[4 * cq] += w.x; park[4 * cq + 1] += w.y; park[4 * cq + 2] += w.z; park[4 * cq + 3] += w.w; }
            }
            add4(gt0, slot); add4(gt1, slot + W4 * 64); add4(gt2, slot + 2 * W4 * 64); add4(gt3, slot + 3 * W4 * 64);
        }
        if (a.park_mode & 2) {
            put4(gt0, slot); put4(gt1, slot + W4 * 64); put4(gt2, slot + 2 * W4 * 64); put4(gt3, slot + 3 * W4 * 64);
            if constexpr (TIES && PARK_REGS) { uint4 *ge_to = slot + 4 * W4 * 64; put4(ge0, ge_to); put4(ge1, ge_to + W4 * 64); put4(ge2, ge_to + 2 * W4 * 64); put4(ge3, ge_to + 3 * W4 * 64); }
            else if constexpr (TIES) {
                uint4 *ge_to = slot + 4 * W4 * 64;
#pragma clang loop unroll(disable)
                for (int cq = 0; cq < 4 * W4; ++cq) ge_to[cq * 64] = uint4{park[4 * cq], park[4 * cq + 1], park[4 * cq + 2], park[4 * cq + 3]};
            }
            if (lane == 0) a.park_ge[idx] = TIES ? 1 : 0;
            return;
        }
    }
    const int g = side ? a.gt : a.gc;
    const int m = side ? a.m2 : a.m1, n = side ? a.nt : a.nc;
#pragma clang loop unroll(disable)
    for (int r = 0; r < ((SLOTS && sep) ? 0 : RJ); ++r) {
        const Counts cur = gt0;
        Counts cge = 0;
        if constexpr (TIES && PARK_REGS) cge = ge0;
        else if constexpr (TIES) {
#pragma unroll
            for (int h = 0; h < RI / 2; ++h) cge[h] = park[r * (RI / 2) + h];
        }
        emit_gene<RI, true, SLOTS>(a, i0, jl + 64 * r, bi, lane, side ? 2 : 0, m, n - m, [&](int ii) {
            const uint32_t w = cur[ii >> 1];
            int nre = static_cast<int>((ii & 1) ? (w >> 16) : (w & 0xFFFFu));
            if (TIES) {
                const uint32_t w2 = cge[ii >> 1];
                const int nge = static_cast<int>((ii & 1) ? (w2 >> 16) : (w2 & 0xFFFFu));
                const bool amb = (nre < m && nge >= m) || (nre <= n - m && nge > n - m);
                if (amb) nre += tie_wins(a.seed, i0 + ii, jl + 64 * r, g, static_cast<uint32_t>(nge - nre));
            }
            return nre;
        });
        gt0 = gt1; gt1 = gt2; gt2 = gt3;
        if constexpr (TIES && PARK_REGS) { ge0 = ge1; ge1 = ge2; ge2 = ge3; }
    }
    if (a.stamps && lane == 0) {
        unsigned long long *st = a.stamps + static_cast<size_t>(idx) * 4;
        st[0] = t_begin; st[1] = t_loop; st[2] = t_emit; st[3] = __builtin_amdgcn_s_memrealtime();
    }
}

template <int NB, bool TIES, bool SLOTS = false>
__device__ __forceinline__ void k1w_body(const K1Args &a, uint4 *ring, uint32_t idx)
{
    constexpr int RI = kTileI, RJ = kRJ;
    const unsigned long long t_begin = a.stamps ? __builtin_amdgcn_s_memrealtime() : 0;
    const uint32_t item = a.items[idx];
    const int jw = __builtin_amdgcn_readfirstlane(static_cast<int>((item >> 16) & 0x7FFFu) * (64 * RJ));
    const int side = __builtin_amdgcn_readfirstlane(static_cast<int>(item >> 31));
    const int tile0 = static_cast<int>(item & 0x3FFFu) * RI;
    if (__builtin_amdgcn_readfirstlane(static_cast<int>(item & 0x8000u))) {
        const int i0 = __builtin_amdgcn_readfirstlane(tile0 + ((item & 0x4000u) ? RI / 2 : 0));
        k1w_item<NB, TIES, RI / 2, SLOTS>(a, ring, idx, i0, jw, side, t_begin);
    } else {
        k1w_item<NB, TIES, RI, SLOTS>(a, ring, idx, __builtin_amdgcn_readfirstlane(tile0), jw, side, t_begin);
    }
}

template <int NB, bool TIES>
__global__ __launch_bounds__(64, NB > 16 ? 2 : 3) void k1w_pairs(K1Args a)
{
    constexpr int RI = kTileI;
    constexpr int ROWB = NB > 16 ? 128 : 64;
    __shared__ uint4 ring[2 * RI * ROWB / 16];
    k1w_body<NB, TIES>(a, ring, blockIdx.x);
}

template <int NB>
__global__ __launch_bounds__(64, 3) void k1w_pairs_slots(K1Args a)
{
    static_assert(NB <= 16, "slot order: 16-bit positions");
    __shared__ uint4 ring[2 * kTileI * 64 / 16];
    const bool pull = a.queue != nullptr;
    const int x = static_cast<int>(blockIdx.x) & (kQueues - 1);
    int s = 0;
#pragma clang loop unroll(disable)
    for (;;) {
        uint32_t idx = blockIdx.x;
        if (pull) {
            bool got = false;
#pragma clang loop unroll(disable)
            while (s < kQueues) {
                const int q = queue_steal(x, s);
                uint32_t m = 0;
                if (threadIdx.x == 0) m = __hip_atomic_fetch_add(a.queue + q * kQueueStride, 1u, __ATOMIC_RELAXED, __HIP_MEMORY_SCOPE_AGENT);
                m = __builtin_amdgcn_readfirstlane(m);
                if (m < queue_len(a.n_items, q)) { idx = queue_index(q, m); got = true; break; }
                ++s;
            }
            if (!got) break;
        }
        k1w_body<NB, false, true>(a, ring, idx);
        if (!pull) break;
    }
}

constexpr int kSlotSplits = 16;
constexpr int kSlotRankSpan = 2048;

__global__ __launch_bounds__(256) void k1_slot_part(const uint16_t *__restrict__ pos16, int Gp, int G, int s0a, int na, int s0b, int nb, uint32_t *__restrict__ part)
{
    const int g = blockIdx.x * 256 + threadIdx.x, split = blockIdx.y, side = blockIdx.z;
    if (g >= G) return;
    const int s0 = side ? s0b : s0a, n = side ? nb : na;
    const int per = (n + kSlotSplits - 1) / kSlotSplits;
    const int b = min(n, split * per), e = min(n, b + per);
    uint32_t mn = kSlotNoMin, mx = kSlotNoMax;
#pragma unroll 4
    for (int s = b; s < e; ++s) {
        const uint32_t v = pos16[static_cast<size_t>(s0 + s) * Gp + g];
        mn = min(mn, v); mx = max(mx, v);
    }
    part[(static_cast<size_t>(split) * 2 + side) * Gp + g] = slot_pack(mn, mx);
}

__global__ __launch_bounds__(256) void k1_slot_keys(const uint32_t *__restrict__ part, int Gp, int G, uint32_t *__restrict__ gmm, uint32_t *__restrict__ key)
{
    const int g = blockIdx.x * 256 + threadIdx.x;
    if (g >= G) return;
    uint32_t r0 = slot_pack(kSlotNoMin, kSlotNoMax), r1 = r0;
#pragma unroll
    for (int y = 0; y < kSlotSplits; ++y) {
        r0 = slot_join(r0, part[(static_cast<size_t>(y) * 2) * Gp + g]);
        r1 = slot_join(r1, part[(static_cast<size_t>(y) * 2 + 1) * Gp + g]);
    }
    gmm[g] = r0; gmm[Gp + g] = r1;
    key[g] = slot_key(r0, r1);
}

__global__ __launch_bounds__(256) void k1_slot_rank(const uint32_t *__restrict__ key, int G, uint32_t *__restrict__ g2s)
{
    __shared__ uint64_t sk[kSlotRankSpan];
    const int h0 = blockIdx.y * kSlotRankSpan;
    for (int t = threadIdx.x; t < kSlotRankSpan; t += 256)
        sk[t] = h0 + t < G ? slot_order_key(key[h0 + t], static_cast<uint32_t>(h0 + t)) : ~0ull;
    __syncthreads();
    const int g = blockIdx.x * 256 + threadIdx.x;
    if (g >= G) return;
    const uint64_t mine = slot_order_key(key[g], static_cast<uint32_t>(g));
    uint32_t n = 0;
#pragma unroll 8
    for (int t = 0; t < kSlotRankSpan; ++t) n += sk[t] < mine ? 1u : 0u;
    if (n) atomicAdd(&g2s[g], n);
}

__global__ __launch_bounds__(256) void k1_slot_invert(uint32_t *__restrict__ g2s, uint32_t *__restrict__ s2g, int G, int Gp)
{
    const int g = blockIdx.x * 256 + threadIdx.x;
    if (g >= Gp) return;
    if (g < G) { const uint32_t k = g2s[g]; if (k < static_cast<uint32_t>(G)) s2g[k] = static_cast<uint32_t>(g); }
    else { g2s[g] = static_cast<uint32_t>(g); s2g[g] = static_cast<uint32_t>(g); }
}

__global__ __launch_bounds__(256) void k1_slot_ranges(const uint32_t *__restrict__ gmm, const uint32_t *__restrict__ s2g, int G, int Gp,
                                                      uint32_t *__restrict__ trng, uint32_t *__restrict__ crng)
{
    static_assert(kSlotTile == kTileI && kSlotChunk == 64 * kRJ, "k1_slots.h carries its own copy of the item geometry");
    __shared__ uint32_t sm[8];
    const int k = blockIdx.x * 256 + threadIdx.x, side = blockIdx.y;
    uint32_t r = k < G ? gmm[static_cast<size_t>(side) * Gp + s2g[k]] : slot_pack(kSlotNoMin, kSlotNoMax);
#pragma unroll
    for (int o = 1; o < 32; o <<= 1) r = slot_join(r, static_cast<uint32_t>(__shfl_xor(static_cast<int>(r), o)));
    if ((threadIdx.x & 31) == 0) { trng[static_cast<size_t>(side) * (Gp >> 5) + (k >> 5)] = r; sm[threadIdx.x >> 5] = r; }
    __syncthreads();
    if (threadIdx.x == 0) {
        for (int q = 1; q < 8; ++q) r = slot_join(r, sm[q]);
        crng[static_cast<size_t>(side) * (Gp >> 8) + blockIdx.x] = r;
    }
}

__global__ __launch_bounds__(256) void k1_slot_gather(const uint4 *__restrict__ P, const uint4 *__restrict__ AL, const uint32_t *__restrict__ s2g, int Gp,
                                                      uint4 *__restrict__ Ps, uint4 *__restrict__ ALs)
{
    const int k = blockIdx.x * 256 + threadIdx.x, b = blockIdx.y;
    const uint32_t g = s2g[k];
#pragma unroll
    for (int q = 0; q < 4; ++q) Ps[(static_cast<size_t>(b) * 4 + q) * Gp + k] = P[(static_cast<size_t>(b) * 4 + q) * Gp + g];
#pragma unroll
    for (int e = 0; e < 4; ++e) {
        const int kk = blockIdx.x * 256 + e * 64 + (threadIdx.x >> 2), q = threadIdx.x & 3;
        ALs[(static_cast<size_t>(b) * Gp + kk) * 4 + q] = AL[(static_cast<size_t>(b) * Gp + s2g[kk]) * 4 + q];
    }
}

template <int R>
__global__ __launch_bounds__(256) void k1_unslot_columns(uint32_t *__restrict__ table, const uint32_t *__restrict__ g2s, int G, int Wp)
{
    extern __shared__ uint4 unslot_sm[];
    uint32_t *sm = reinterpret_cast<uint32_t *>(unslot_sm);
    const int r0 = blockIdx.x * R, nr = min(R, G - r0);
    if (nr <= 0) return;
    uint32_t *rows = table + static_cast<size_t>(r0) * kPlanes * Wp;
    for (int rp = 0; rp < nr * kPlanes; ++rp)
        for (int w = threadIdx.x; w < Wp; w += 256) sm[(static_cast<size_t>(rp >> 2) * Wp + w) * 4 + (rp & 3)] = rows[static_cast<size_t>(rp) * Wp + w];
    __syncthreads();
    for (int wo = threadIdx.x; wo < Wp; wo += 256) {
        uint32_t acc[R][4];
#pragma unroll
        for (int r = 0; r < R; ++r) acc[r][0] = acc[r][1] = acc[r][2] = acc[r][3] = 0;
        const uint4 *kq = reinterpret_cast<const uint4 *>(g2s) + static_cast<size_t>(wo) * 8;
#pragma unroll 2
        for (int i = 0; i < 8; ++i) {
            const uint4 k4 = kq[i];
            const uint32_t ks[4] = {k4.x, k4.y, k4.z, k4.w};
#pragma unroll
            for (int e = 0; e < 4; ++e) {
                const uint32_t k = ks[e], kw = min(k >> 5, static_cast<uint32_t>(Wp - 1)), kb = k & 31u;
#pragma unroll
                for (int r = 0; r < R; ++r) {
                    if (r < nr) {
                        const uint4 w = unslot_sm[static_cast<size_t>(r) * Wp + kw];
                        acc[r][0] = __builtin_amdgcn_alignbit(w.x >> kb, acc[r][0], 1);
                        acc[r][1] = __builtin_amdgcn_alignbit(w.y >> kb, acc[r][1], 1);
                        acc[r][2] = __builtin_amdgcn_alignbit(w.z >> kb, acc[r][2], 1);
                        acc[r][3] = __builtin_amdgcn_alignbit(w.w >> kb, acc[r][3], 1);
                    }
                }
            }
        }
        const int left = G - 32 * wo;
        const uint32_t valid = left >= 32 ? 0xFFFFFFFFu : (left <= 0 ? 0u : (1u << left) - 1u);
#pragma unroll
        for (int r = 0; r < R; ++r)
            if (r < nr) {
#pragma unroll
                for (int pl = 0; pl < 4; ++pl) rows[(static_cast<size_t>(r) * kPlanes + pl) * Wp + wo] = acc[r][pl] & valid;
            }
    }
}

template <int R>
__global__ __launch_bounds__(kUnslotThreadsMax) void k1_unslot_words(uint32_t *__restrict__ table, const uint32_t *__restrict__ g2s, int G, int Wp)
{
    constexpr int NQ = 4 * R;
    extern __shared__ uint32_t unslot_t[];
    const int r0 = blockIdx.x * R, nr = min(R, G - r0);
    if (nr <= 0) return;
    const int nq = nr * kPlanes;
    uint32_t *rows = table + static_cast<size_t>(r0) * kPlanes * Wp;
    for (int w = threadIdx.x; w < Wp; w += blockDim.x) {
        uint32_t m[NQ];
#pragma unroll
        for (int q = 0; q < NQ; ++q) m[q] = q < nq ? rows[static_cast<size_t>(q) * Wp + w] : 0u;
        unslot_in_word<R>(m, w, unslot_t);
    }
    __syncthreads();
    for (int wo = threadIdx.x; wo < Wp; wo += blockDim.x) {
        const uint4 *kq = reinterpret_cast<const uint4 *>(g2s) + static_cast<size_t>(wo) * 8;
        uint32_t ks[32], u[NQ];
#pragma unroll
        for (int i = 0; i < 8; ++i) {
            const uint4 k4 = kq[i];
            ks[4 * i] = k4.x; ks[4 * i + 1] = k4.y; ks[4 * i + 2] = k4.z; ks[4 * i + 3] = k4.w;
        }
        unslot_out_word<R>(u, ks, wo, unslot_t, G, 32 * Wp);
#pragma unroll
        for (int q = 0; q < NQ; ++q)
            if (q < nq) rows[static_cast<size_t>(q) * Wp + wo] = u[q];
    }
}

__global__ __launch_bounds__(256) void k1_slot_count(const uint32_t *__restrict__ items, int n, const uint32_t *__restrict__ trng, const uint32_t *__restrict__ crng,
                                                     int Gp, unsigned long long *__restrict__ out)
{
    const int i = blockIdx.x * 256 + threadIdx.x;
    int v = 0;
    if (i < n) {
        const uint32_t it = items[i];
        const int side = slot_item_side(it);
        if (slot_separated(trng[static_cast<size_t>(side) * (Gp >> 5) + slot_item_tile(it)], crng[static_cast<size_t>(side) * (Gp >> 8) + slot_item_chunk(it)]))
            v = slot_item_halves(it);
    }
    const unsigned long long m1 = __ballot(v == 1), m2 = __ballot(v == 2);
    if ((threadIdx.x & 63) == 0 && (m1 | m2)) atomicAdd(out, static_cast<unsigned long long>(__builtin_popcountll(m1) + 2 * __builtin_popcountll(m2)));
}

template <int NB>
__global__ __launch_bounds__(64, NB > 16 ? 2 : 3) void k1w_pairs_gated(K1Args a)
{
    constexpr int RI = kTileI;
    constexpr int ROWB = NB > 16 ? 128 : 64;
    __shared__ uint4 ring[2 * RI * ROWB / 16];
    const int bad = a.gate[0] | a.gate[4] | a.gate[5], ties = a.gate[1];
    if (bad) return;
    if (ties) k1w_body<NB, true>(a, ring, blockIdx.x);
    else k1w_body<NB, false>(a, ring, blockIdx.x);
}

constexpr int kRJWide = 2, kRJWideTies = 1;

template <int RJ, int NB, bool TIES>
__device__ __forceinline__ void count_pass_wide(const uint4 *__restrict__ P, const uint4 *__restrict__ AL, const uint4 *__restrict__ AH,
                                                int Gp, int i0, int jl, int bb, int be, uint32_t (&gt)[RJ][kTileI],
                                                uint32_t (&ge)[TIES ? RJ : 1][kTileI], uint4 *sm_lo, uint4 *sm_hi, bool idle)
{
    static_assert((TIES && RJ == 1) || (!TIES && RJ == 2), "four chains per bit plane");
    constexpr int RI = kTileI, NQ = (NB + 3) / 4;
    constexpr int kStageQ = kStageB * RI * 4;
    constexpr int kPerThread = kStageQ / 256;
#pragma unroll
    for (int r = 0; r < RJ; ++r)
#pragma unroll
        for (int ii = 0; ii < RI; ++ii) { gt[r][ii] = 0; if (TIES) ge[r][ii] = 0; }
    if (bb >= be) return;
    uint4 sl[kPerThread], sh[TIES ? kPerThread : 1];
    auto stage_load = [&](int b0) {
#pragma unroll
        for (int e = 0; e < kPerThread; ++e) {
            const int idx = threadIdx.x + 256 * e;
            const int b = min(b0 + idx / (RI * 4), be - 1);
            const size_t o = (static_cast<size_t>(b) * Gp + i0) * 4 + idx % (RI * 4);
            sl[e] = AL[o];
            if (TIES) sh[e] = AH[o];
        }
    };
    auto stage_store = [&](int buf) {
#pragma unroll
        for (int e = 0; e < kPerThread; ++e) {
            sm_lo[buf * kStageQ + threadIdx.x + 256 * e] = sl[e];
            if (TIES) sm_hi[buf * kStageQ + threadIdx.x + 256 * e] = sh[e];
        }
    };
    stage_load(bb);
    __syncthreads();
    stage_store(0);
    __syncthreads();
    int buf = 0;
    for (int b0 = bb; b0 < be; b0 += kStageB) {
        const bool more = b0 + kStageB < be;
        if (more) stage_load(b0 + kStageB);
        const int nb = idle ? 0 : min(kStageB, be - b0);
        for (int s = 0; s < nb; ++s) {
            Planes16 p[RJ];
#pragma unroll
            for (int r = 0; r < RJ; ++r)
#pragma unroll
                for (int q = 0; q < NQ; ++q) p[r].set(q, P[(static_cast<size_t>(b0 + s) * 4 + q) * Gp + jl + 64 * r]);
            const uint4 *al = sm_lo + buf * kStageQ + s * RI * 4;
            const uint4 *ah = sm_hi + buf * kStageQ + s * RI * 4;
#pragma clang loop unroll(full)
            for (int i = 0; i < RI; i += 2) {
                Planes16 a0, a1, c0, c1;
#pragma unroll
                for (int q = 0; q < 4; ++q) {
                    if (q < 3 && 4 * q + 1 > NB - 1) continue;
                    a0.set(q, al[i * 4 + q]); a1.set(q, al[(i + 1) * 4 + q]);
                    if (TIES) { c0.set(q, ah[i * 4 + q]); c1.set(q, ah[(i + 1) * 4 + q]); }
                }
                uint32_t l[4];
                if (TIES) {
                    chains_first(l, p[0].w[0], p[0].w[0], p[0].w[0], p[0].w[0], a0.w[a_word(0)], c0.w[a_word(0)], a1.w[a_word(0)], c1.w[a_word(0)]);
#pragma unroll
                    for (int k = 1; k < NB; ++k)
                        chains_next(l, p[0].w[k], p[0].w[k], p[0].w[k], p[0].w[k], a0.w[a_word(k)], c0.w[a_word(k)], a1.w[a_word(k)], c1.w[a_word(k)]);
                    gt[0][i] += __builtin_popcount(l[0]); ge[0][i] += __builtin_popcount(l[1]);
                    gt[0][i + 1] += __builtin_popcount(l[2]); ge[0][i + 1] += __builtin_popcount(l[3]);
                } else {
                    chains_first(l, p[0].w[0], p[RJ - 1].w[0], p[0].w[0], p[RJ - 1].w[0], a0.w[a_word(0)], a0.w[a_word(0)], a1.w[a_word(0)], a1.w[a_word(0)]);
#pragma unroll
                    for (int k = 1; k < NB; ++k)
                        chains_next(l, p[0].w[k], p[RJ - 1].w[k], p[0].w[k], p[RJ - 1].w[k], a0.w[a_word(k)], a0.w[a_word(k)], a1.w[a_word(k)], a1.w[a_word(k)]);
                    gt[0][i] += __builtin_popcount(l[0]); gt[RJ - 1][i] += __builtin_popcount(l[1]);
                    gt[0][i + 1] += __builtin_popcount(l[2]); gt[RJ - 1][i + 1] += __builtin_popcount(l[3]);
                }
            }
        }
        if (more) stage_store(buf ^ 1);
        __syncthreads();
        buf ^= 1;
    }
}

template <int NB, bool TIES, bool MULTI>
__global__ __launch_bounds__(256, 2) void k1_pairs_wide(K1Args a)
{
    constexpr int RI = kTileI, RJ = TIES ? kRJWideTies : kRJWide;
    int i0, jl;
    if (!tile_of_block<RI, RJ>(a, i0, jl)) return;
    const int lane = threadIdx.x & 63, bi = i0 >> 6;
    __shared__ uint4 sm_lo[2 * kStageB * RI * 4];
    __shared__ uint4 sm_hi[TIES ? 2 * kStageB * RI * 4 : 1];
    const bool idle = wave_idle<RJ>(jl & ~63, i0, a.G);
    uint32_t gt[RJ][RI], ge[TIES ? RJ : 1][RI];
    auto count_of = [&](int r, int ii, int g) -> int {
        int nre = static_cast<int>(gt[r][ii]);
        if (TIES) {
            const uint32_t neq = ge[r][ii] - gt[r][ii];
            if (neq) nre += tie_wins(a.seed, i0 + ii, jl + 64 * r, g, neq);
        }
        return nre;
    };
    count_pass_wide<RJ, NB, TIES>(a.P, a.AL, a.AH, a.Gp, i0, jl, a.cb, a.ce, gt, ge, sm_lo, sm_hi, idle);
    emit_side<RI, RJ>(a, i0, jl, bi, lane, 0, a.m1, a.nc - a.m1, [&](int r, int ii) { return count_of(r, ii, a.gc); });
    if (!MULTI) {
        count_pass_wide<RJ, NB, TIES>(a.P, a.AL, a.AH, a.Gp, i0, jl, a.tb, a.te, gt, ge, sm_lo, sm_hi, idle);
        emit_side<RI, RJ>(a, i0, jl, bi, lane, 2, a.m2, a.nt - a.m2, [&](int r, int ii) { return count_of(r, ii, a.gt); });
    } else {
        int tot[RJ][RI];
#pragma unroll
        for (int r = 0; r < RJ; ++r)
#pragma unroll
            for (int ii = 0; ii < RI; ++ii) tot[r][ii] = 0;
        for (int g = 0; g < a.ngroups; ++g) {
            if (g == a.gc) continue;
            count_pass_wide<RJ, NB, TIES>(a.P, a.AL, a.AH, a.Gp, i0, jl, a.goff[g], a.goff[g + 1], gt, ge, sm_lo, sm_hi, idle);
#pragma unroll
            for (int r = 0; r < RJ; ++r)
#pragma unroll
                for (int ii = 0; ii < RI; ++ii) tot[r][ii] += count_of(r, ii, g);
        }
        emit_side<RI, RJ>(a, i0, jl, bi, lane, 2, a.m2, a.nt - a.m2, [&](int r, int ii) { return tot[r][ii]; });
// ... 2734 lines not shown
    if (!c->xs) {
        for (int q = 0; q < 2; ++q) REO_HIP_CHECK(handle_stream(&c->k1s[q], 0));
        REO_HIP_CHECK(handle_stream(&c->xs, 0));
        REO_HIP_CHECK(handle_event(&c->ev_fork, 0));
        REO_HIP_CHECK(handle_event(&c->ev_x, 0));
        for (int q = 0; q < 2; ++q) REO_HIP_CHECK(handle_event(&c->ev_k1_join[q], 0));
        for (int q = 0; q < 8; ++q) REO_HIP_CHECK(handle_event(&c->ev_k1[q], 0));
    }
    std::vector<std::vector<uint32_t>> wunits(nwaves);
    for (size_t m = 0; m < units.size(); ++m) wunits[std::min<size_t>(m / mw, nwaves - 1)].push_back(units[m]);
    for (int w = 0; w < nwaves; ++w)
        if ((rc = item_list(c, a, pl, 3, wunits[w], c->k1_wave_items[w], w, nwaves))) return rc;
    if ((rc = upload_units_all(c))) return rc;
    if (!c->table_prezeroed) REO_HIP_CHECK(hipMemsetAsync(c->table.p, 0, static_cast<size_t>(c->G) * kPlanes * c->Wp * sizeof(uint32_t), c->stream));
    c->table_prezeroed = false;
    c->last_k1_shared = 0;
    tic(c, 1);
    int32_t xrc = REO_OK;
    auto hip_ok = [&](hipError_t e, const char *what) {
        if (e == hipSuccess || xrc) return e == hipSuccess;
        set_error("%s failed: %s (pipelined exchange)", what, hipGetErrorString(e));
        xrc = e == hipErrorOutOfMemory ? REO_ENOMEM : REO_EHIP;
        return false;
    };
    bool forked = hip_ok(hipEventRecord(c->ev_fork, c->stream), "hipEventRecord(fork)");
    for (int q = 0; q < 2 && forked; ++q) forked = hip_ok(hipStreamWaitEvent(c->k1s[q], c->ev_fork, 0), "hipStreamWaitEvent(fork)");
    if (forked) forked = hip_ok(hipStreamWaitEvent(c->xs, c->ev_fork, 0), "hipStreamWaitEvent(fork)");
    for (int w = 0; w < nwaves && !xrc; ++w) {
        hipStream_t ks = c->k1s[w & 1];
        dispatch_wave(w, ks);
        if (!hip_ok(hipGetLastError(), "pair kernel launch")) break;
        if (!hip_ok(hipEventRecord(c->ev_k1[w], ks), "hipEventRecord(wave)") || !hip_ok(hipStreamWaitEvent(c->xs, c->ev_k1[w], 0), "hipStreamWaitEvent(wave)")) break;
        const int m0 = w * mw, mc = std::max(0, std::min(mw, maxu_x - m0));
        if (mc == 0) continue;
        uint32_t *send = c->xsend.p + uw * mw * w, *recv = c->xrecv.p + uw * mw * w * c->world;
        const int64_t bytes = static_cast<int64_t>(uw) * mc * sizeof(uint32_t);
        if ((xrc = launch_pack_units(c, m0, mc, send, c->xs))) break;
        if (c->comm) { if ((xrc = comm_allgather(c, send, recv, bytes, c->xs)) < 0) break; xrc = REO_OK; }
        else {
            const int hrc = c->ag(send, recv, bytes, c->xs, c->ag_user);
            if (hrc) { set_error("all-gather hook failed with %d", hrc); xrc = REO_ECOMM; break; }
        }
        if ((xrc = launch_expand_units(c, m0, mc, recv, c->xs))) break;
    }
    bool joined = true;
    for (int q = 0; q < 2; ++q)
        if (hipEventRecord(c->ev_k1_join[q], c->k1s[q]) != hipSuccess || hipStreamWaitEvent(c->stream, c->ev_k1_join[q], 0) != hipSuccess) joined = false;
    toc(c);
    tic(c, 6);
    if (hipEventRecord(c->ev_x, c->xs) != hipSuccess || hipStreamWaitEvent(c->stream, c->ev_x, 0) != hipSuccess) joined = false;
    toc(c);
    if (!joined) {
        for (int q = 0; q < 2; ++q) (void)hipStreamSynchronize(c->k1s[q]);
        (void)hipStreamSynchronize(c->xs);
        if (!xrc) { set_error("joining the streams of the pipelined exchange failed"); xrc = REO_EHIP; }
    }
    if (xrc) return xrc;
    c->x_pipelined = true;
    return REO_OK;
}

static int32_t report_k1_stamps(reo_ctx *c, unsigned long long *stamps)
{
    std::vector<unsigned long long> h(c->k1_items_n * 4 + 2);
    REO_HIP_CHECK(hipMemcpyAsync(h.data(), stamps, h.size() * sizeof(unsigned long long), hipMemcpyDeviceToHost, c->stream));
    REO_HIP_CHECK(hipStreamSynchronize(c->stream));
    double pro = 0, loop = 0, emit = 0;
    unsigned long long t0 = ~0ull, t1 = 0;
    for (size_t i = 0; i < c->k1_items_n; ++i) {
        pro += static_cast<double>(h[4 * i + 1] - h[4 * i]); loop += static_cast<double>(h[4 * i + 2] - h[4 * i + 1]);
        emit += static_cast<double>(h[4 * i + 3] - h[4 * i + 2]);
        t0 = std::min(t0, h[4 * i]); t1 = std::max(t1, h[4 * i + 3]);
    }
    const double n = static_cast<double>(c->k1_items_n) * 100.0;
    fprintf(stderr, "[reo] K1 wave items %zu: prologue %.2f us, count loop %.2f us, classification %.2f us per item; first start to last end %.3f ms\n",
            c->k1_items_n, pro / n, loop / n, emit / n, static_cast<double>(t1 - t0) / 1e5);
    fprintf(stderr, "[reo]   a launch before it ended %.1f us before the first item began; one after it began %.1f us after the last item ended\n",
            static_cast<double>(static_cast<long long>(t0 - h[c->k1_items_n * 4])) / 100.0, static_cast<double>(static_cast<long long>(h[c->k1_items_n * 4 + 1] - t1)) / 100.0);
    constexpr int kSl = 24;
    const double span = static_cast<double>(t1 - t0) + 1.0;
    double busy[kSl] = {}, dur[kSl] = {};
    size_t started[kSl] = {};
    for (size_t i = 0; i < c->k1_items_n; ++i) {
        const double b = static_cast<double>(h[4 * i] - t0), e = static_cast<double>(h[4 * i + 3] - t0);
        const int s0 = static_cast<int>(b / span * kSl);
        started[s0]++; dur[s0] += static_cast<double>(h[4 * i + 2] - h[4 * i + 1]);
        for (int s = s0; s < kSl; ++s) {
            const double lo = span * s / kSl, hi = span * (s + 1) / kSl;
            if (e <= lo) break;
            busy[s] += (std::min(e, hi) - std::max(b, lo)) / (hi - lo);
        }
    }
    fprintf(stderr, "[reo]   items in flight by slice:");
    for (int s = 0; s < kSl; ++s) fprintf(stderr, " %.0f", busy[s]);
    fprintf(stderr, "\n[reo]   loop us of items started in slice:");
    for (int s = 0; s < kSl; ++s) fprintf(stderr, " %.0f", started[s] ? dur[s] / static_cast<double>(started[s]) / 100.0 : 0.0);
    fprintf(stderr, "\n");
    (void)hipFree(stamps);
    return REO_OK;
}

static K1Args k1_args(const reo_ctx *c, int k)
{
    K1Args a;
    a.P = c->pos.p; a.AL = c->lo.p; a.AH = c->hi.p; a.table = c->table.p;
    a.G = static_cast<int>(c->G); a.Gp = c->Gp; a.Wp = c->Wp;
    const bool multi = c->ngroups > 2;
    const int other = multi ? k : 1 - k;
    a.cb = c->goff32[k] / 32; a.ce = c->goff32[k + 1] / 32;
    a.tb = c->goff32[other] / 32; a.te = c->goff32[other + 1] / 32;
    a.gc = k; a.gt = other;
    a.nc = c->goff[k + 1] - c->goff[k]; a.nt = static_cast<int>(c->S) - a.nc;
    a.goff = c->goff_dev.p; a.ngroups = c->ngroups;
    a.m1 = c->thr[2 * k]; a.m2 = c->thr[2 * k + 1];
    a.seed = c->seed;
    a.items = nullptr; a.stamps = nullptr; a.gate = nullptr;
    a.park = nullptr; a.park_ge = nullptr; a.park_mode = 0;
    a.s2g = nullptr; a.trng = nullptr; a.crng = nullptr;
    a.queue = nullptr; a.n_items = 0;
    return a;
}

static int32_t upload_unit_map(reo_ctx *c, const std::vector<uint32_t> &units)
{
    int32_t rc;
    if ((rc = c->unit_map.ensure(std::max<size_t>(units.size(), 1)))) return rc;
    if (!units.empty() && (c->unit_map.p != c->unit_map_uploaded || units != c->unit_map_host)) {
        REO_HIP_CHECK(hipMemcpyAsync(c->unit_map.p, units.data(), units.size() * sizeof(uint32_t), hipMemcpyHostToDevice, c->stream));
        REO_HIP_CHECK(hipStreamSynchronize(c->stream));
        c->unit_map_host = units;
        c->unit_map_uploaded = c->unit_map.p;
    }
    return REO_OK;
}

static int32_t apply_range(reo_ctx *c, K1Args &a, int sides, const K1Range *range, size_t n_items)
{
    int32_t rc;
    const int side = sides == 1 ? 0 : 1, sb = side ? a.tb : a.cb, se = side ? a.te : a.ce;
    if (range->b0 < 0 || range->b1 <= range->b0 || sb + range->b1 > se || (range->first != (range->b0 == 0)) || (range->last != (sb + range->b1 == se))) {
        set_error("a range of sample blocks outside its side"); return REO_EINVAL;
    }
    if (!(range->first && range->last)) {
        if ((rc = c->k1_park[side].ensure(std::max<size_t>(n_items, 1) * kParkSlot)) || (rc = c->k1_park_ge[side].ensure(std::max<size_t>(n_items, 1)))) return rc;
        a.park = c->k1_park[side].p; a.park_ge = c->k1_park_ge[side].p;
        a.park_mode = (range->first ? 0 : 1) | (range->last ? 0 : 2);
    }
    (side ? a.tb : a.cb) = sb + range->b0;
    (side ? a.te : a.ce) = sb + range->b1;
    return REO_OK;
}


struct SlotMaps { uint32_t *gmm, *key, *g2s, *s2g, *trng, *crng; unsigned long long *count; };
static size_t slot_maps_words(int Gp) { return static_cast<size_t>(Gp) * 5 + static_cast<size_t>(Gp) / 16 + static_cast<size_t>(Gp) / 128 + 2; }
static SlotMaps slot_maps(const reo_ctx *c)
{
    SlotMaps m;
    const size_t Gp = static_cast<size_t>(c->Gp);
    m.gmm = c->k1_slot_maps.p; m.key = m.gmm + 2 * Gp; m.g2s = m.key + Gp; m.s2g = m.g2s + Gp;
    m.trng = m.s2g + Gp; m.crng = m.trng + Gp / 16;
    m.count = reinterpret_cast<unsigned long long *>(m.crng + Gp / 128);
    return m;
}

static bool k1_slots_wanted(const reo_ctx *c, const K1Plan &pl, int sides, bool keep_table, const int32_t *gate, const K1Range *range, bool prepare)
{
    return c->k1_slots && pl.wave && !pl.wide && !pl.big && c->ngroups == 2 && sides == 3 && !c->has_ties && c->world == 1 && !c->in_multi &&
           !gate && !range && !prepare && !keep_table && c->t_pos16.p && c->t_pos16.n >= static_cast<size_t>(c->goff32[2]) * c->Gp;
}

static int32_t k1_slots_alloc(reo_ctx *c)
{
    int32_t rc;
    const size_t nq = static_cast<size_t>(c->goff32[2] / 32) * c->Gp * 4;
    if ((rc = c->k1_slot_part.ensure(static_cast<size_t>(kSlotSplits) * 2 * c->Gp)) || (rc = c->k1_slot_maps.ensure(slot_maps_words(c->Gp))) ||
        (rc = c->pos_s.ensure(nq)) || (rc = c->lo_s.ensure(nq)))
        return rc;
    if (c->k1_queue && c->k1_queue_ctr.ensure(kQueueWords)) (void)hipGetLastError();
    return REO_OK;
}

static int32_t k1_slots_front(reo_ctx *c, K1Args &a)
{
    const int G = a.G, Gp = a.Gp, nblk = c->goff32[2] / 32;
    const SlotMaps m = slot_maps(c);
    const unsigned gb = static_cast<unsigned>((G + 255) / 256);
    REO_HIP_CHECK(hipMemsetAsync(m.g2s, 0, static_cast<size_t>(Gp) * 2 * sizeof(uint32_t), c->stream));
    k1_slot_part<<<dim3(gb, kSlotSplits, 2), 256, 0, c->stream>>>(c->t_pos16.p, Gp, G, a.cb * 32, a.nc, a.tb * 32, a.nt, c->k1_slot_part.p);
    k1_slot_keys<<<gb, 256, 0, c->stream>>>(c->k1_slot_part.p, Gp, G, m.gmm, m.key);
    k1_slot_rank<<<dim3(gb, static_cast<unsigned>((G + kSlotRankSpan - 1) / kSlotRankSpan)), 256, 0, c->stream>>>(m.key, G, m.g2s);
    k1_slot_invert<<<static_cast<unsigned>(Gp / 256), 256, 0, c->stream>>>(m.g2s, m.s2g, G, Gp);
    k1_slot_ranges<<<dim3(static_cast<unsigned>(Gp / 256), 2), 256, 0, c->stream>>>(m.gmm, m.s2g, G, Gp, m.trng, m.crng);
    k1_slot_gather<<<dim3(static_cast<unsigned>(Gp / 256), static_cast<unsigned>(nblk)), 256, 0, c->stream>>>(c->pos.p, c->lo.p, m.s2g, Gp, c->pos_s.p, c->lo_s.p);
    REO_HIP_CHECK(hipGetLastError());
    a.P = c->pos_s.p; a.AL = c->lo_s.p; a.AH = c->lo_s.p;
    a.s2g = m.s2g; a.trng = m.trng; a.crng = m.crng;
    a.n_items = static_cast<uint32_t>(c->k1_items_n);
    if (c->k1_queue && c->k1_queue_ctr.p && c->k1_queue_ctr.n >= static_cast<size_t>(kQueueWords)) {
        REO_HIP_CHECK(hipMemsetAsync(c->k1_queue_ctr.p, 0, kQueueWords * sizeof(uint32_t), c->stream));
        a.queue = c->k1_queue_ctr.p;
    }
    return REO_OK;
}

static int32_t k1_slots_back(reo_ctx *c, const K1Args &a)
{
    if (c->k1_unslot != 0) {
        int form = unslot_form(a.Gp);
        if ((c->k1_unslot == kUnslotWide || c->k1_unslot == kUnslotNarrow) && unslot_lds_bytes(c->k1_unslot, a.Gp) <= kUnslotLdsLimit) form = c->k1_unslot;
        const size_t lds = unslot_lds_bytes(form, a.Gp);
        if (lds <= kUnslotLdsLimit) {
            auto go = [&](auto rtag) -> int32_t {
                constexpr int R = decltype(rtag)::value;
                const int bit = R == kUnslotWide ? 1 : 2;
                if (!(c->k1_unslot_attr & bit)) {
                    REO_HIP_CHECK(hipFuncSetAttribute(reinterpret_cast<const void *>(k1_unslot_words<R>), hipFuncAttributeMaxDynamicSharedMemorySize, static_cast<int>(kUnslotLdsLimit)));
                    c->k1_unslot_attr |= bit;
                }
                k1_unslot_words<R><<<static_cast<unsigned>((a.G + R - 1) / R), static_cast<unsigned>(unslot_threads(a.Wp)), lds, c->stream>>>(a.table, slot_maps(c).g2s, a.G, a.Wp);
                return REO_OK;
            };
            const int32_t rc = form == kUnslotWide ? go(std::integral_constant<int, kUnslotWide>{}) : go(std::integral_constant<int, kUnslotNarrow>{});
            if (rc) return rc;
            REO_HIP_CHECK(hipGetLastError());
            c->last_k1_unslot = form;
            return REO_OK;
        }
    }
    c->last_k1_unslot = 1;
    const size_t row_bytes = static_cast<size_t>(a.Wp) * 16;
    auto go = [&](auto rtag) {
        constexpr int R = decltype(rtag)::value;
        k1_unslot_columns<R><<<static_cast<unsigned>((a.G + R - 1) / R), 256, R * row_bytes, c->stream>>>(a.table, slot_maps(c).g2s, a.G, a.Wp);
    };
    if (6 * row_bytes <= 61440) go(std::integral_constant<int, 6>{});
    else if (4 * row_bytes <= 61440) go(std::integral_constant<int, 4>{});
    else if (2 * row_bytes <= 61440) go(std::integral_constant<int, 2>{});
    else go(std::integral_constant<int, 1>{});
    REO_HIP_CHECK(hipGetLastError());
    return REO_OK;
}

int32_t launch_slot_separated(reo_ctx *c, int64_t *half_tiles)
{
    *half_tiles = 0;
    if (!c->last_k1_slots || !c->k1_slot_items || !c->k1_slot_items_n || !c->k1_slot_maps.p) return REO_OK;
    const reo_ctx::ItemList &il = c->k1_wave_items[0];
    if (c->k1_slot_gp != c->Gp || c->k1_slot_maps.n < slot_maps_words(c->Gp) || c->k1_slot_items != il.buf.p || c->k1_slot_items_n > il.buf.n) return REO_OK;
    const SlotMaps m = slot_maps(c);
    unsigned long long n = 0;
    REO_HIP_CHECK(hipMemsetAsync(m.count, 0, sizeof n, c->stream));
    k1_slot_count<<<static_cast<unsigned>((c->k1_slot_items_n + 255) / 256), 256, 0, c->stream>>>(c->k1_slot_items, static_cast<int>(c->k1_slot_items_n), m.trng, m.crng, c->Gp, m.count);
    REO_HIP_CHECK(hipGetLastError());
    REO_HIP_CHECK(hipMemcpyAsync(&n, m.count, sizeof n, hipMemcpyDeviceToHost, c->stream));
    REO_HIP_CHECK(hipStreamSynchronize(c->stream));
    *half_tiles = static_cast<int64_t>(n);
    return REO_OK;
}

int32_t launch_k1(reo_ctx *c, int k, int sides, bool keep_table, const int32_t *gate, const K1Range *range, bool prepare, int treat)
{
    K1Args a = k1_args(c, k);
    K1Plan pl;
    int32_t rc;
    if (treat >= 0) {
        if (sides != 3 || keep_table || gate || range || prepare || c->ngroups <= 2) { set_error("a contrast of two groups: more than two groups, the whole table"); return REO_EINVAL; }
        const ContrastSides cs = contrast_sides(c->goff.data(), c->goff32.data(), c->thr.data(), k, treat);
        a.cb = cs.cb; a.ce = cs.ce; a.tb = cs.tb; a.te = cs.te;
        a.gc = k; a.gt = treat;
        a.nc = cs.nc; a.nt = cs.nt; a.m1 = cs.m1; a.m2 = cs.m2;
        pl.contrast = true;
    }
    if ((rc = k1_plan(c, sides, pl))) return rc;
    const std::vector<uint32_t> &units = pl.units;
    c->units_all_host = pl.units_all;
    c->tiles_owned = pl.tiles_owned; c->tiles_total = pl.tiles_total;
    c->k1_cj = pl.CJ; c->k1_q = pl.Q;
    a.n_units = static_cast<int>(units.size()); a.Q = pl.Q;
    if ((rc = upload_unit_map(c, units))) return rc;
    a.unit_map = c->unit_map.p;
    a.gate = gate;
    if (!prepare) { c->last_k1_slots = 0; c->k1_slot_items = nullptr; c->k1_slot_items_n = 0; c->k1_slot_gp = 0; }
    if ((range || prepare) && (sides != 1 && sides != 2)) { set_error("a range of sample blocks / a prepared launch: one side of the pair kernel"); return REO_EINVAL; }
    if (gate && (!pl.wave || pl.wide || pl.big)) { set_error("a gated launch of the pair kernel: wave form, at most 65535 genes and samples"); return REO_EINVAL; }
    c->x_pipelined = false;
    const int maxu_x = exchange_units_per_rank(c);
    const int nwaves = (pl.wave && sides == 3 && c->world > 1 && (c->comm || c->ag) && !c->in_multi && !c->k1_stamps) ? std::min({c->x_waves, 8, maxu_x}) : 1;
    if (nwaves > 1) {
        hipStream_t main_stream = c->stream;
        return pipelined_exchange(c, a, pl, nwaves, maxu_x, [&](int w, hipStream_t ks) {
            c->stream = ks;
            a.items = c->k1_wave_items[w].buf.p; c->k1_items_n = c->k1_wave_items[w].n;
            if (c->k1_items_n) dispatch_pairs(c, a, pl);
            c->stream = main_stream;
        });
    }
    if (pl.wave || (pl.wcounts && !c->gc_valid) || pl.wmulti) {
        reo_ctx::ItemList &il = c->k1_wave_items[sides == 3 ? 0 : sides];
        const auto w0 = std::chrono::steady_clock::now();
        if ((rc = item_list(c, a, pl, sides, units, il, 0, 1))) return rc;
        if (c->debug_passes) fprintf(stderr, "  launch_k1 sides %d: item list (%zu items) ready after %.0f us\n", sides, il.n, std::chrono::duration<double, std::micro>(std::chrono::steady_clock::now() - w0).count());
        a.items = il.buf.p; c->k1_items_n = il.n;
        if (prepare) return REO_OK;
        if (range && (rc = apply_range(c, a, sides, range, il.n))) return rc;
        if (c->k1_stamps) REO_HIP_CHECK(hipMalloc(reinterpret_cast<void **>(&a.stamps), (std::max<size_t>(c->k1_items_n, 1) * 4 + 2) * sizeof(unsigned long long)));
    }
    if (!keep_table) {
        if (!c->table_prezeroed) REO_HIP_CHECK(hipMemsetAsync(c->table.p, 0, static_cast<size_t>(c->G) * kPlanes * c->Wp * sizeof(uint32_t), c->stream));
        c->table_prezeroed = false;
    }
    if (units.empty()) return REO_OK;
    c->last_k1_shared = pl.shared ? 1 : 0;
    if (k1_slots_wanted(c, pl, sides, keep_table, gate, range, prepare) && c->k1_items_n) {
        if (k1_slots_alloc(c) == REO_OK) pl.slots = true;
        else (void)hipGetLastError();
    }
    if (a.stamps) k_time_mark<<<1, 64, 0, c->stream>>>(a.stamps + c->k1_items_n * 4);
    tic(c, 1);
    if (pl.slots && (rc = k1_slots_front(c, a))) { toc(c); return rc; }
    dispatch_pairs(c, a, pl);
    if (pl.slots && (rc = k1_slots_back(c, a))) { toc(c); return rc; }
    toc(c);
    if (pl.slots) {
        c->last_k1_slots = 1;
        c->k1_slot_items = a.items; c->k1_slot_items_n = c->k1_items_n; c->k1_slot_gp = a.Gp;
    }
    if (a.stamps) k_time_mark<<<1, 64, 0, c->stream>>>(a.stamps + c->k1_items_n * 4 + 1);
    REO_HIP_CHECK(hipGetLastError());
    if (a.stamps) return report_k1_stamps(c, a.stamps);
    return REO_OK;
}


int64_t exchange_unit_words(const reo_ctx *c) { return static_cast<int64_t>(kUnitRows) * kPlanes * (c->k1_q * c->k1_cj / 32); }
int32_t exchange_units_per_rank(const reo_ctx *c)
{
    const int total = static_cast<int>(c->units_all_host.size()), world = std::max(c->world, 1);
    return std::max(1, (total + world - 1) / world);
}

static int32_t upload_units_all(reo_ctx *c)
{
    int32_t rc;
    const size_t total = c->units_all_host.size();
    if ((rc = c->units_all.ensure(std::max<size_t>(total, 1)))) return rc;
    if (total && (c->units_all.p != c->units_all_uploaded || c->units_all_host != c->units_all_dev)) {
        REO_HIP_CHECK(hipMemcpyAsync(c->units_all.p, c->units_all_host.data(), total * sizeof(uint32_t), hipMemcpyHostToDevice, c->stream));
        REO_HIP_CHECK(hipStreamSynchronize(c->stream));
        c->units_all_dev = c->units_all_host;
        c->units_all_uploaded = c->units_all.p;
    }
    return REO_OK;
}

static int32_t exchange_args(reo_ctx *c, XArgs &a, int m0, int mcnt)
{
    const int32_t rc = upload_units_all(c);
    if (rc) return rc;
    a.table = c->table.p; a.units = c->units_all.p;
    a.G = static_cast<int>(c->G); a.Wp = c->Wp; a.Wc = c->k1_q * c->k1_cj / 32;
    a.total = static_cast<int>(c->units_all_host.size()); a.world = std::max(c->world, 1); a.rank = c->rank; a.maxu = exchange_units_per_rank(c);
    a.m0 = m0; a.mcnt = mcnt < 0 ? a.maxu : mcnt;
    return REO_OK;
}

int32_t launch_pack_units(reo_ctx *c, int m0, int mcnt, uint32_t *send, hipStream_t st)
{
    XArgs a;
    int32_t rc = exchange_args(c, a, m0, mcnt);
    if (rc) return rc;
    const size_t uw = static_cast<size_t>(exchange_unit_words(c));
    x_pack<<<dim3(static_cast<unsigned>((uw + 255) / 256), a.mcnt), 256, 0, st ? st : c->stream>>>(a, send ? send : c->xsend.p);
    REO_HIP_CHECK(hipGetLastError());
    return REO_OK;
}

int32_t launch_expand_units(reo_ctx *c, int m0, int mcnt, const uint32_t *recv, hipStream_t st)
{
    XArgs a;
    int32_t rc = exchange_args(c, a, m0, mcnt);
    if (rc) return rc;
    if (a.world < 2) return REO_OK;
    const size_t uw = static_cast<size_t>(exchange_unit_words(c));
    if (!st) st = c->stream;
    if (!recv) recv = c->xrecv.p;
    x_expand_fwd<<<dim3(static_cast<unsigned>((uw + 255) / 256), a.mcnt * a.world), 256, 0, st>>>(a, recv);
    x_expand_mirror<<<dim3(a.Wc, kPlanes, a.mcnt * a.world), 256, 0, st>>>(a, recv);
    REO_HIP_CHECK(hipGetLastError());
    return REO_OK;
}

int32_t launch_counts(reo_ctx *c, int64_t i0, int64_t i1, int64_t j0, int64_t j1, uint16_t *d_gt, uint16_t *d_eq)
{
    dim3 grid(static_cast<unsigned>((j1 - j0 + 255) / 256), static_cast<unsigned>(i1 - i0));
    if (c->G > 65535)
        k1_counts_big<<<grid, 256, 0, c->stream>>>(c->pos.p, c->lo.p, c->hi.p, c->Gp, plane_bits(c->G), c->goff_dev.p, c->ngroups,
                                                   static_cast<int>(i0), static_cast<int>(i1), static_cast<int>(j0), static_cast<int>(j1), d_gt, d_eq);
    else
        k1_counts<<<grid, 256, 0, c->stream>>>(c->pos.p, c->lo.p, c->hi.p, c->Gp, plane_bits(c->G), c->goff_dev.p, c->ngroups,
                                               static_cast<int>(i0), static_cast<int>(i1), static_cast<int>(j0), static_cast<int>(j1), d_gt, d_eq);
    REO_HIP_CHECK(hipGetLastError());
    return REO_OK;
}

int32_t launch_check_table(reo_ctx *c, int *bad)
{
    *bad = 0;
    int32_t rc = c->check_flag.ensure(1);
    if (rc) return rc;
    REO_HIP_CHECK(hipMemsetAsync(c->check_flag.p, 0, sizeof(int32_t), c->stream));
    const int G = static_cast<int>(c->G);
    k_check_table<<<(G + 3) / 4, 256, 0, c->stream>>>(c->table.p, G, c->Wp, c->check_flag.p);
    int32_t h = 0;
    REO_HIP_CHECK(hipMemcpyAsync(&h, c->check_flag.p, sizeof h, hipMemcpyDeviceToHost, c->stream));
    REO_HIP_CHECK(hipStreamSynchronize(c->stream));
    *bad = h;
    return REO_OK;
}

int32_t launch_decode(reo_ctx *c, int64_t i0, int64_t i1, int64_t j0, int64_t j1, uint8_t *d_code)
{
    dim3 grid(static_cast<unsigned>((j1 - j0 + 255) / 256), static_cast<unsigned>(i1 - i0));
    k_decode<<<grid, 256, 0, c->stream>>>(c->table.p, c->Wp, static_cast<int>(i0), static_cast<int>(i1),
                                          static_cast<int>(j0), static_cast<int>(j1), d_code);
    REO_HIP_CHECK(hipGetLastError());
    return REO_OK;
}

int32_t launch_pack_ref(reo_ctx *c, const uint8_t *d_bytes, uint32_t *d_bits)
{
    k_pack_ref<<<c->Gp / 256, 256, 0, c->stream>>>(d_bytes, c->Gp, d_bits);
    REO_HIP_CHECK(hipGetLastError());
    return REO_OK;
}

__global__ void k_cycle_skip(IterState *st, IterState *host_st, int32_t *trace, int skip, int period)
{
    const int T = st->passes;
    for (int u = T + static_cast<int>(threadIdx.x); u < T + skip; u += static_cast<int>(blockDim.x)) {
        const int src = T - period + (u - T) % period;
        trace[2 * u] = trace[2 * src]; trace[2 * u + 1] = trace[2 * src + 1];
    }
    __syncthreads();
    if (threadIdx.x != 0) return;
    st->passes = T + skip;
    if (st->raw_pass >= 0) st->raw_pass += skip;
    st->i_iter += skip;
    st->cyc_period = -1;
    if (host_st) { host_st->passes = T + skip; host_st->cyc_period = -1; }
}

int32_t launch_cycle_skip(reo_ctx *c, int skip, int period)
{
    if (skip < 0 || period < 1 || skip % period != 0 || (skip & 1)) { set_error("launch_cycle_skip: skip %d, period %d", skip, period); return REO_EINVAL; }
    k_cycle_skip<<<1, 256, 0, c->stream>>>(c->state.p, c->state_mirror ? c->host_state : nullptr, c->trace.p, skip, period);
    REO_HIP_CHECK(hipGetLastError());
    return REO_OK;
}

int32_t launch_iter_init(reo_ctx *c, const uint8_t *host_ref, const IterState *host_state)
{
    IterInitArgs a;
    a.host_ref = host_ref; a.host_state = reinterpret_cast<const uint32_t *>(host_state);
    a.refbytes = c->refbytes[0].p; a.refbits = c->refbits[0].p; a.state = reinterpret_cast<uint32_t *>(c->state.p);
    a.zero[0] = reinterpret_cast<uint32_t *>(c->result.p); a.zero_n[0] = static_cast<size_t>(c->G) * 15 * 2;
    a.zero[1] = reinterpret_cast<uint32_t *>(c->modes.p); a.zero_n[1] = c->modes.n;
    a.zero[2] = reinterpret_cast<uint32_t *>(c->hist.p); a.zero_n[2] = c->hist.n;
    a.G = static_cast<int>(c->G); a.Gp = c->Gp; a.state_words = static_cast<int>(sizeof(IterState) / 4);
    k_iter_init<<<c->Gp / 256, 256, 0, c->stream>>>(a);
    REO_HIP_CHECK(hipGetLastError());
    return REO_OK;
}

int32_t launch_tally(reo_ctx *c, int nref)
{
    const int G = static_cast<int>(c->G);
    tic(c, 2);
// ... 141 lines not shown
```

### rankcompv3.jl_amd/csrc/reo_internal.h

```cpp
#pragma once

#include <hip/hip_runtime.h>

#include <cstdint>
#include <functional>
#include <string>
#include <vector>

#include "reo_hip.h"

namespace reo {

constexpr int kTileJ = 256;
constexpr int kTileI = 32;
constexpr int kPlanes = 4;
constexpr int kUnitH = 32;
constexpr int kRJ = 4;
constexpr int kRJTies = 2;
constexpr int kMaxGenes = 262143;
constexpr int kGenePad = 1024;
constexpr int kRaw = 8;
constexpr int kDeltaMax = 128;
constexpr int kSortChunk = 1024;

// ... 53 lines not shown
};
struct LightSlot {
    LightRec rec;
    int32_t bfail;
    int32_t cdiff;
    int32_t cfound;
    int32_t pad0[5];
    double wnext[4];
    double se_base;
    double eta;
    double pad1[15];
    LightCnt lc;
};
struct LightState { LightSlot slot[kLightBatch + 2]; };
static_assert(sizeof(LightSlot) % 128 == 0, "LightSlot layout");

void set_error(const char *fmt, ...);

#define REO_HIP_CHECK(expr)                                                              \
    do {                                                                                 \
        hipError_t e_ = (expr);                                                          \
        if (e_ != hipSuccess) {                                                          \
            ::reo::set_error("%s failed: %s (%s:%d)", #expr, hipGetErrorString(e_),      \
                             __FILE__, __LINE__);                                        \
            return e_ == hipErrorOutOfMemory ? REO_ENOMEM : REO_EHIP;                    \
        }                                                                                \
    } while (0)

hipError_t pool_alloc(void **p, size_t bytes, bool pinned);
void pool_free(void *p, size_t bytes, bool pinned);
extern thread_local bool tl_release_synced;
hipError_t handle_stream(hipStream_t *s, int kind);
hipError_t handle_event(hipEvent_t *e, int kind);
void release_stream(hipStream_t s, int kind);
void release_event(hipEvent_t e, int kind);

template <class T>
struct DevBuf {
    T *p = nullptr;
    size_t n = 0;
    DevBuf() = default;
    DevBuf(const DevBuf &) = delete;
    DevBuf &operator=(const DevBuf &) = delete;
    ~DevBuf() { release(); }
    int32_t ensure(size_t count)
    {
        if (count <= n && p) return REO_OK;
        release();
        REO_HIP_CHECK(pool_alloc(reinterpret_cast<void **>(&p), count * sizeof(T), false));
        n = count;
        return REO_OK;
    }
    void release()
    {
        if (p) {
            if (!tl_release_synced) (void)hipDeviceSynchronize();
            pool_free(p, n * sizeof(T), false);
        }
        p = nullptr;
        n = 0;
    }
};

struct StageTimer {
    hipEvent_t a = nullptr, b = nullptr;
};

}

struct reo_ctx {
    int device = 0;
    hipStream_t stream = nullptr;
    uint64_t seed = 0;
    int rank = 0, world = 1;
    reo_allreduce_fn ar = nullptr;
    void *ar_user = nullptr;
    reo_allgather_fn ag = nullptr;
    void *ag_user = nullptr;

    int64_t G = 0, S = 0, ld = 0;
    int dtype = 0;
    const void *dX = nullptr;
    reo::DevBuf<unsigned char> dX_owned;
    std::vector<int32_t> group_id;
    int ngroups = 0;
    std::vector<int32_t> thr;
    bool thr_set = false;

    int Gp = 0, Wp = 0;
    std::vector<int32_t> goff;
    std::vector<int32_t> goff32;
    reo::DevBuf<uint4> pos;
    reo::DevBuf<uint4> lo;
    reo::DevBuf<uint4> hi;
    reo::DevBuf<uint16_t> t_pos16, t_lo16, t_hi16;
    reo::DevBuf<uint32_t> t_pos32, t_lo32, t_hi32;
    reo::DevBuf<uint32_t> t_vin32, t_vout32;
    reo::DevBuf<int32_t> goff_dev;
    reo::DevBuf<uint64_t> t_kin, t_kout;
    reo::DevBuf<uint16_t> t_vin, t_vout;
    reo::DevBuf<unsigned char> t_temp;
    reo::DevBuf<int32_t> t_order, t_flags, t_slots;
    reo::DevBuf<uint32_t> unit_map;
    std::vector<uint32_t> unit_map_host;
    std::vector<int32_t> t_order_host, t_slots_host, goff_blocks_host;
    const int32_t *t_meta_ptr[3] = {nullptr, nullptr, nullptr};
    int32_t *host_flags = nullptr;
    hipEvent_t ev_flags = nullptr;
    bool table_prezeroed = false;
    const uint32_t *unit_map_uploaded = nullptr;
    size_t k1_items_n = 0;
    bool transformed = false;
    int eager_mode = 2;
    int eager_chunk = 0;
    int eager_gate = 1;
    hipStream_t up = nullptr, rk = nullptr;
    hipEvent_t ev_up[8] = {nullptr};
    hipEvent_t ev_rk[4] = {nullptr, nullptr, nullptr, nullptr};
    reo::DevBuf<int32_t> e_lists;
    int upload_threads = 12;
    unsigned char *stage_h[3] = {nullptr, nullptr, nullptr};
    size_t stage_cap = 0;
    reo::DevBuf<unsigned char> stage_d[3];
    hipEvent_t ev_stage[3] = {nullptr, nullptr, nullptr}, ev_widen[3] = {nullptr, nullptr, nullptr};
    int64_t narrowed_bytes = 0;
    int rowmajor_upload = 0;
    int csc_upload = 0;
    int64_t csc_nnz = 0;
    reo::DevBuf<int64_t> csc_colptr;
    int csc_device = 0;
    bool eager_k1 = false;
    int has_ties = 0;
    int transform_in_lds = 0;

    reo::DevBuf<uint32_t> table;
    int built_k = -1;
    int built_treat = -1;
    bool table_complete = false;
    void *comm = nullptr;
    int spin_wait = 0;
    int check_hook_table = 1;
    bool comm_dead = false;
    bool in_multi = false;
    bool multi_one_device = false;
    std::vector<reo_ctx *> peers;
    reo::DevBuf<uint16_t> gcounts;
    bool gc_valid = false;
    int k1_wave = 1;
    int k1_order = 0;
    int k1_half = 1;
    int k1_slots = 1;
    int last_k1_slots = 0;
    int k1_unslot = -1;
    int last_k1_unslot = 0;
    int k1_unslot_attr = 0;
    const uint32_t *k1_slot_items = nullptr;
    size_t k1_slot_items_n = 0;
    int k1_slot_gp = 0;
    reo::DevBuf<uint32_t> k1_slot_part;
    reo::DevBuf<uint32_t> k1_slot_maps;
    reo::DevBuf<uint4> pos_s, lo_s;
    int k1_queue = 1;
    int k1_workers = 0;
    reo::DevBuf<uint32_t> k1_queue_ctr;
    int n_cus = 256;
    int share_counts = 1;
    int last_k1_shared = 0;
    int64_t tiles_owned = 0, tiles_total = 0;
    int k1_cj = 0, k1_q = 0;
    std::vector<uint32_t> units_all_host, units_all_dev;
    const uint32_t *units_all_uploaded = nullptr;
    reo::DevBuf<uint32_t> units_all, xsend, xrecv;
    int x_waves = 4;
    bool x_pipelined = false;
    hipStream_t k1s[2] = {nullptr, nullptr}, xs = nullptr;
    hipEvent_t ev_fork = nullptr, ev_k1[8] = {nullptr}, ev_k1_join[2] = {nullptr, nullptr}, ev_x = nullptr;
    struct ItemList { reo::DevBuf<uint32_t> buf; size_t n = 0; uint64_t key[5] = {0, 0, 0, 0, 0}; };
    ItemList k1_wave_items[8];
    reo::DevBuf<uint32_t> k1_park[2];
    reo::DevBuf<int32_t> k1_park_ge[2];
    int64_t eager_range_launches = 0;
    int eager_ranges = -1;
    reo::DevBuf<int32_t> check_flag;

    reo::DevBuf<uint32_t> refbits[2];
    reo::DevBuf<uint8_t> refbytes[2];
    int ref_slot = -1;
    const char *ref_gone = "reo_identify_degs has not run on this context";
    reo::DevBuf<int32_t> sc_slot2col;
    std::vector<int32_t> sc_slot2col_host;
    const int32_t *sc_slot2col_uploaded = nullptr;
    reo::DevBuf<double> st_lf;
    int64_t st_lf_G = -1;
    reo::DevBuf<int32_t> raw;
    reo::DevBuf<uint32_t> delta_list;
    reo::DevBuf<int32_t> cont;
    reo::DevBuf<double> result;
    reo::DevBuf<double> sorted_d;
    reo::DevBuf<double> sorted_p;
    reo::DevBuf<uint32_t> rank_s, rank_a;
    reo::DevBuf<double> scal;
    reo::DevBuf<double> blockmin;
    reo::DevBuf<double> chunk_v;
    reo::DevBuf<uint16_t> chunk_i;
    reo::DevBuf<double> part;
    reo::DevBuf<reo::IterState> state;
    reo::DevBuf<int32_t> trace;
    reo::DevBuf<int32_t> modes;
    reo::DevBuf<double> cand;
    reo::DevBuf<unsigned> gridbar;
    reo::DevBuf<reo::LightState> lstate;
    reo::DevBuf<int32_t> clist;
    int light_band = 32;
    bool cycle_watch = true;
    reo::DevBuf<uint8_t> snap;
    int it_cycle_period = 0, it_cycle_at = 0, it_cycle_skipped = 0;
    int hist_below = 256;
    int xcc_local = 0;
    int light_window = 24, light_min_g = 4096;
    int light_mode = 1;
    reo::DevBuf<int32_t> olist;
    reo::DevBuf<int32_t> hist, mrank;
    double it_pval_deg = 1.0, it_padj_deg = 0.05;
    int it_n_iter = 0, it_n_conv = 0, it_a0 = 0, it_b0 = 0;
    int k2_idx = 0;
    int it_light_form = 1;
    bool it_no_light = false;
    reo::IterState *host_state = nullptr;
    bool state_mirror_wanted = true;
    bool debug_passes = false, debug_stamps = false, k1_stamps = false;
    bool state_mirror = false;
    uint8_t *host_ref = nullptr;
    size_t host_ref_cap = 0;

    bool profiling = false;
    double t_ms[REO_NTIMINGS] = {0};
    std::vector<std::pair<int, reo::StageTimer>> pending;
    std::vector<reo::StageTimer> pool;
    std::vector<size_t> open;
    std::vector<int32_t> k2_modes;
    size_t k2_seen = 0;
};

namespace reo {

int32_t run_transform(reo_ctx *c);
enum { kLayoutColMajor = 0, kLayoutRowMajor = 1, kLayoutCsc = 2 };
int32_t eager_upload(reo_ctx *c, const void *hX, int64_t hld, bool with_k1, bool host_i32 = false, int layout = kLayoutColMajor);
int32_t upload_columns(reo_ctx *c, const void *hX, int64_t hld, int64_t G, int64_t ncols, void *dX, int dtype, int layout = kLayoutColMajor);
int32_t widen_device_i32(reo_ctx *c, const void *dX32, int64_t ld, int64_t G, int64_t S, void *dX64);
int32_t densify_device_csc(reo_ctx *c, int64_t G, int64_t S, const int64_t *colptr, const void *rows, int32_t index_bits, const void *vals,
                           int dtype, void *dX);
int32_t ensure_upload_streams(reo_ctx *c);
int32_t ensure_staging(reo_ctx *c, size_t slot_bytes);
void host_parallel(int nthreads, int ntasks, const std::function<void(int)> &fn);

struct K1Range { int b0, b1; bool first, last; };
int32_t launch_k1(reo_ctx *c, int k, int sides = 3, bool keep_table = false, const int32_t *gate = nullptr, const K1Range *range = nullptr,
                  bool prepare = false, int treat = -1);
int32_t k1_planes_fit(reo_ctx *c, bool *fit, size_t *need_bytes);
int64_t exchange_unit_words(const reo_ctx *c);
int32_t exchange_units_per_rank(const reo_ctx *c);
int32_t launch_pack_units(reo_ctx *c, int m0 = 0, int mcnt = -1, uint32_t *send = nullptr, hipStream_t st = nullptr);
int32_t launch_expand_units(reo_ctx *c, int m0 = 0, int mcnt = -1, const uint32_t *recv = nullptr, hipStream_t st = nullptr);
int32_t launch_slot_separated(reo_ctx *c, int64_t *half_tiles);
int32_t launch_counts(reo_ctx *c, int64_t i0, int64_t i1, int64_t j0, int64_t j1, uint16_t *d_gt, uint16_t *d_eq);
int32_t launch_check_table(reo_ctx *c, int *bad);
int32_t launch_decode(reo_ctx *c, int64_t i0, int64_t i1, int64_t j0, int64_t j1, uint8_t *d_code);
int32_t launch_pack_ref(reo_ctx *c, const uint8_t *d_bytes, uint32_t *d_bits);
int32_t launch_cycle_skip(reo_ctx *c, int skip, int period);
int32_t launch_iter_init(reo_ctx *c, const uint8_t *host_ref, const IterState *host_state);
int32_t launch_tally(reo_ctx *c, int nref);
int32_t launch_full_pass(reo_ctx *c, bool replay);
int32_t launch_light_persistent(reo_ctx *c);
int32_t launch_light_batch(reo_ctx *c, int nlight);
int32_t xcc_selftest(reo_ctx *c, int *ok);
int32_t light_min_genes();
int32_t light_window();
int32_t launch_mccullagh(reo_ctx *c, const int32_t *d_cont, int64_t n, double *d_out);

int32_t launch_pair_count(reo_ctx *c, const int32_t *d_genes, int64_t n_genes, const uint32_t *d_maskbits, uint32_t class_mask, int32_t *d_count);
int32_t launch_pair_fill(reo_ctx *c, const int32_t *d_genes, int64_t n_genes, const uint32_t *d_maskbits, uint32_t class_mask, const int64_t *d_rowptr,
                         int32_t *d_partner, uint8_t *d_code, int64_t capacity, int32_t *d_flag);

int plane_bits(int64_t G);
int32_t launch_sample_counts(reo_ctx *c, const int32_t *d_genes, int64_t n_queries, const uint32_t *d_maskbits, uint32_t class_mask,
                             const int32_t *d_slot2col, int32_t *d_sel, int32_t *d_gt, int32_t *d_eq);

int32_t launch_sample_fisher(reo_ctx *c, int64_t n_queries, const int32_t *d_sel_a, const int32_t *d_sel_b, const int32_t *d_gt_a,
                             const int32_t *d_eq_a, const int32_t *d_gt_b, const int32_t *d_eq_b, const double *d_lf, int64_t lf_entries,
                             int32_t *d_rev_up, int32_t *d_rev_down, int32_t *d_tied, double *d_p_up, double *d_p_down, int32_t *d_flag);

int32_t launch_call_rank(reo_ctx *c, int64_t n_genes, int64_t q0, int64_t nq, const double *d_p_up, const double *d_p_down, double pval_deg,
                         double padj_deg, uint32_t *d_words);
int32_t launch_call_cut(reo_ctx *c, int64_t n_genes, const uint32_t *d_words, int32_t *d_kstar, int32_t *d_cut, int32_t *d_n_up, int32_t *d_n_down);
int32_t launch_call_emit(reo_ctx *c, int64_t n_genes, const uint32_t *d_words, const int32_t *d_kstar, int8_t *d_calls);

struct PsItem;
int32_t launch_pair_support(reo_ctx *c, const PsItem *d_items, int64_t n_items, const int32_t *d_partner, const int32_t *d_slot2col,
                            int32_t *d_gt, int32_t *d_eq, uint8_t *d_outcome);

int32_t pseudobulk_resident_dense(reo_ctx *c, const void *X, bool is_int, int64_t G, int64_t C, int64_t ld, const int32_t *order,
                                  int64_t n_order, const int32_t *chunk_ptr, int32_t n_out);
int32_t pseudobulk_resident_csc(reo_ctx *c, bool is_int, int64_t G, int64_t C, const int64_t *colptr, const int32_t *rowidx, const void *val,
                                const int32_t *order, int64_t n_order, const int32_t *chunk_ptr, int32_t n_out);
int32_t pseudobulk_device_dense(reo_ctx *c, int dtype, const void *dX, int64_t G, int64_t C, int64_t ld, const int32_t *order, int64_t n_order,
// ... 40 lines not shown
```

Baseline: 48900 billion.

## Give each sample side its own slot order and sort-based slot ranking

Each side of the pair kernel can now get its own gene slot permutation, keyed by that side's min+max rank window, instead of one common key. The slot, range, gather and un-permute stages are made side-aware, and a paired un-permute kernel is added. The O(G*span) rank count is replaced by a bitonic sort per span followed by a binary-search rank, with a 32-bit key path when there are at most 32768 genes. Per-side orders are meant to tighten the tile/chunk ranges so more pair tiles are found separable and skipped, but they cost extra map memory and a second sort/invert pass.

```diff
diff --git a/rankcompv3.jl_amd/_ffi.py b/rankcompv3.jl_amd/_ffi.py
--- a/rankcompv3.jl_amd/_ffi.py
+++ b/rankcompv3.jl_amd/_ffi.py
@@ -825,8 +825,8 @@
                 "k2_full_launches": int(ms[9]), "k2_delta_ms": ms[10], "set_matrix_host_wall_ms": ms[11]}
 
     def info(self) -> dict:
-        w = np.zeros(30, dtype=np.int64)
-        check(self._L.reo_get_info(self._h, _ptr(w), 30))
+        w = np.zeros(31, dtype=np.int64)
+        check(self._L.reo_get_info(self._h, _ptr(w), 31))
         v = np.zeros(28, dtype=np.int64)
         v[:] = w[:28]
         return {"G": int(v[0]), "S": int(v[1]), "Gp": int(v[2]), "table_bytes": int(v[3]), "has_ties": int(v[4]),
@@ -837,4 +837,4 @@
                 "eager_range_launches": int(v[20]), "rowmajor_upload": int(v[21]),
                 "csc_upload": int(v[22]), "csc_nnz": int(v[23]), "resident_dtype": int(v[24]),
                 "k1_slot_order": int(v[25]), "k1_half_tiles_separated": int(v[26]), "csc_device": int(v[27]),
-                "k1_unslot_form": int(w[28]), "contrast_treat": int(w[29])}
+                "k1_unslot_form": int(w[28]), "contrast_treat": int(w[29]), "k1_slot_sides": int(w[30])}
diff --git a/rankcompv3.jl_amd/csrc/api.hip b/rankcompv3.jl_amd/csrc/api.hip
--- a/rankcompv3.jl_amd/csrc/api.hip
+++ b/rankcompv3.jl_amd/csrc/api.hip
@@ -333,7 +333,7 @@
     c->built_treat = -1;
     c->gc_valid = false;
     c->eager_k1 = false;
-    c->last_k1_slots = 0; c->k1_slot_items = nullptr; c->k1_slot_items_n = 0; c->k1_slot_gp = 0;
+    c->last_k1_slots = 0; c->last_k1_slot_sides = 0; c->k1_slot_items = nullptr; c->k1_slot_items_n = 0; c->k1_slot_gp = 0;
 }
 
 static size_t elem_bytes(int dtype) { return dtype >= 3 ? 4 : 8; }
@@ -616,6 +616,7 @@
     if (const char *e = getenv("REO_K1_SLOTS")) c->k1_slots = (e[0] != '0');
     if (const char *e = getenv("REO_K1_QUEUE")) c->k1_queue = (e[0] != '0');
     if (const char *e = getenv("REO_K1_UNSLOT")) { const int v = atoi(e); c->k1_unslot = (v == 8 || v == 4) ? v : (e[0] == '0' ? 0 : -1); }
+    if (const char *e = getenv("REO_K1_SLOT_SIDES")) { const int v = atoi(e); c->k1_slot_sides = (v == 1 || v == 2) ? v : 0; }
     if (const char *e = getenv("REO_K1_WORKERS")) c->k1_workers = std::max(1, atoi(e));
     if (const char *e = getenv("REO_K1_ORDER")) c->k1_order = std::max(0, std::min(2, atoi(e)));
     {
@@ -1383,15 +1384,16 @@
         int32_t rc = use(c);
         if (rc || (rc = launch_slot_separated(c, &separated))) return rc;
     }
-    const int64_t v[30] = {c->G, c->S, c->Gp, static_cast<int64_t>(c->table.n * sizeof(uint32_t)), c->has_ties,
+    const int64_t v[31] = {c->G, c->S, c->Gp, static_cast<int64_t>(c->table.n * sizeof(uint32_t)), c->has_ties,
                            c->tiles_owned, c->tiles_total, kTileI, c->k1_cj, c->k1_q, kUnitH,
                            c->goff32.empty() ? 0 : c->goff32.back(), c->last_k1_shared,
                            static_cast<int64_t>(c->gcounts.n * sizeof(uint16_t)), c->transform_in_lds, c->xcc_local,
                            c->it_cycle_period, c->it_cycle_at, c->it_cycle_skipped, c->narrowed_bytes, c->eager_range_launches, c->rowmajor_upload,
                            c->csc_upload, c->csc_nnz, c->dtype, c->last_k1_slots, separated, c->csc_device,
-                           c->last_k1_slots ? c->last_k1_unslot : 0, c->built_k >= 0 ? c->built_treat : -1};
-    for (int i = 0; i < n && i < 30; ++i) info[i] = v[i];
-    return REO_OK;
-}
-
-}
+                           c->last_k1_slots ? c->last_k1_unslot : 0, c->built_k >= 0 ? c->built_treat : -1,
+                           c->last_k1_slots ? c->last_k1_slot_sides : 0};
+    for (int i = 0; i < n && i < 31; ++i) info[i] = v[i];
+    return REO_OK;
+}
+
+}
diff --git a/rankcompv3.jl_amd/csrc/k1_slots.h b/rankcompv3.jl_amd/csrc/k1_slots.h
--- a/rankcompv3.jl_amd/csrc/k1_slots.h
+++ b/rankcompv3.jl_amd/csrc/k1_slots.h
@@ -28,6 +28,19 @@
 
 REO_SLOTS_HD uint64_t slot_order_key(uint32_t key, uint32_t gene) { return static_cast<uint64_t>(key) << 32 | gene; }
 
+REO_SLOTS_HD uint32_t slot_side_key(uint32_t side) { return slot_min(side) + slot_max(side); }
+
+constexpr int kSlotKey32Genes = 32768;
+REO_SLOTS_HD bool slot_order_key32_fits(int G) { return G <= kSlotKey32Genes; }
+REO_SLOTS_HD uint32_t slot_order_key32(uint32_t key, uint32_t gene) { return key << 15 | gene; }
+
+constexpr int kSlotSidesBlocks = 16;
+REO_SLOTS_HD int slot_sides_wanted(int blocks0, int blocks1, int force)
+{
+    if (force == 1 || force == 2) return force;
+    return blocks0 + blocks1 >= kSlotSidesBlocks ? 2 : 1;
+}
+
 REO_SLOTS_HD int slot_separated(uint32_t tile_rng, uint32_t chunk_rng)
 {
     if (slot_max(chunk_rng) < slot_min(tile_rng)) return 1;
@@ -54,6 +67,37 @@
 {
     for (int g = 0; g < G; ++g) { g2s[g] = g2s_G[g]; s2g[g2s_G[g]] = static_cast<uint32_t>(g); }
     for (int g = G; g < Gp; ++g) g2s[g] = s2g[g] = static_cast<uint32_t>(g);
+}
+
+inline void slot_rank32(const uint32_t *key, int G, uint32_t *g2s)
+{
+    for (int g = 0; g < G; ++g) {
+        uint32_t n = 0;
+        for (int h = 0; h < G; ++h) n += slot_order_key32(key[h], static_cast<uint32_t>(h)) < slot_order_key32(key[g], static_cast<uint32_t>(g)) ? 1u : 0u;
+        g2s[g] = n;
+    }
+}
+
+inline void slot_maps_sides(const uint32_t *gmm, int G, int Gp, uint32_t *key, uint32_t *g2s, uint32_t *s2g, uint32_t *rank_G)
+{
+    for (int z = 0; z < 2; ++z) {
+        const size_t o = static_cast<size_t>(z) * Gp;
+        for (int g = 0; g < G; ++g) key[o + g] = slot_side_key(gmm[o + g]);
+        if (slot_order_key32_fits(G)) slot_rank32(key + o, G, rank_G);
+        else slot_rank(key + o, G, rank_G);
+        slot_invert(rank_G, G, Gp, g2s + o, s2g + o);
+    }
+}
+
+inline void slot_ranges_side(const uint32_t *gmm_z, const uint32_t *s2g_z, int G, int Gp, uint32_t *trng, uint32_t *crng)
+{
+    for (int t = 0; t < Gp / kSlotTile; ++t) trng[t] = slot_pack(kSlotNoMin, kSlotNoMax);
+    for (int q = 0; q < Gp / kSlotChunk; ++q) crng[q] = slot_pack(kSlotNoMin, kSlotNoMax);
+    for (int k = 0; k < G; ++k) {
+        const uint32_t r = gmm_z[s2g_z[k]];
+        trng[k / kSlotTile] = slot_join(trng[k / kSlotTile], r);
+        crng[k / kSlotChunk] = slot_join(crng[k / kSlotChunk], r);
+    }
 }
 
 inline void slot_unpermute_row(const uint32_t *in, uint32_t *out, int W, const uint32_t *g2s, int G)
@@ -171,6 +215,28 @@
     }
 }
 
+REO_SLOTS_HD int unslot_pair_bit(int row, int plane) { return 2 * row + plane; }
+REO_SLOTS_HD size_t unslot_pair_word(int q, int side, int Wp, int w) { return (static_cast<size_t>(q >> 1) * 4 + 2 * side + (q & 1)) * Wp + w; }
+
+template <int R>
+inline void unslot_pair_model(uint32_t *table, int r0, int n_rows, int side, int G, int Wp, const uint32_t *g2s, uint32_t *T)
+{
+    const int nr = n_rows - r0 < 2 * R ? n_rows - r0 : 2 * R;
+    if (nr <= 0) return;
+    uint32_t *rows = table + static_cast<size_t>(r0) * 4 * Wp;
+    for (int w = 0; w < Wp; ++w) {
+        uint32_t m[4 * R];
+        for (int q = 0; q < 4 * R; ++q) m[q] = q < 2 * nr ? rows[unslot_pair_word(q, side, Wp, w)] : 0u;
+        unslot_in_word<R>(m, w, T);
+    }
+    for (int wo = 0; wo < Wp; ++wo) {
+        uint32_t u[4 * R], ks[32];
+        for (int c = 0; c < 32; ++c) ks[c] = g2s[32 * wo + c];
+        unslot_out_word<R>(u, ks, wo, T, G, 32 * Wp);
+        for (int q = 0; q < 2 * nr; ++q) rows[unslot_pair_word(q, side, Wp, wo)] = u[q];
+    }
+}
+
 inline void slot_permute_row(const uint32_t *in, uint32_t *out, int W, const uint32_t *s2g, int G)
 {
     for (int w = 0; w < W; ++w) out[w] = 0;
diff --git a/rankcompv3.jl_amd/csrc/kernels.hip b/rankcompv3.jl_amd/csrc/kernels.hip
--- a/rankcompv3.jl_amd/csrc/kernels.hip
+++ b/rankcompv3.jl_amd/csrc/kernels.hip
@@ -255,7 +255,7 @@
     else emit_rows<RI, 0>(near, d, lanes_ok, hi_thr, lo_thr, wL, wH, fLlo, fLhi, fHlo, fHhi, val);
     const bool diag = (bj == bi);
     if (lane < RI && i0 + lane < a.G) {
-        const size_t gi = SLOTS ? a.s2g[i0 + lane] : static_cast<size_t>(i0 + lane);
+        const size_t gi = SLOTS ? a.s2g[(pl >> 1) * a.Gp + i0 + lane] : static_cast<size_t>(i0 + lane);
         uint32_t *row = a.table + (gi * kPlanes + pl) * a.Wp + 2 * bj;
         if (!diag) {
             *reinterpret_cast<uint2 *>(row) = uint2{fLlo, fLhi};
@@ -268,7 +268,7 @@
         }
     }
     if (j < a.G) {
-        const size_t gj = SLOTS ? a.s2g[j] : static_cast<size_t>(j);
+        const size_t gj = SLOTS ? a.s2g[(pl >> 1) * a.Gp + j] : static_cast<size_t>(j);
         uint32_t *row = a.table + (gj * kPlanes + pl) * a.Wp + (i0 >> 5);
         if (RI == 16) {
             const int half = (i0 >> 4) & 1;
@@ -299,7 +299,8 @@
     else if (n <= lo_thr) ++mir;
     else return;
     const bool row_ok = lane < RI && i0 + lane < a.G;
-    uint32_t *frow = a.table + (static_cast<size_t>(row_ok ? a.s2g[i0 + lane] : 0u) * kPlanes + fwd) * a.Wp;
+    const uint32_t *s2g = a.s2g + side * a.Gp;
+    uint32_t *frow = a.table + (static_cast<size_t>(row_ok ? s2g[i0 + lane] : 0u) * kPlanes + fwd) * a.Wp;
 #pragma unroll
     for (int r = 0; r < kRJ; ++r) {
         const int j = jl + 64 * r;
@@ -309,7 +310,7 @@
         if (!lanes_ok) continue;
         if (row_ok) *reinterpret_cast<uint2 *>(frow + 2 * bj) = uint2{static_cast<uint32_t>(lanes_ok), static_cast<uint32_t>(lanes_ok >> 32)};
         if (j < a.G) {
-            uint32_t *row = a.table + (static_cast<size_t>(a.s2g[j]) * kPlanes + mir) * a.Wp + (i0 >> 5);
+            uint32_t *row = a.table + (static_cast<size_t>(s2g[j]) * kPlanes + mir) * a.Wp + (i0 >> 5);
             if (RI == 16) reinterpret_cast<uint16_t *>(row)[(i0 >> 4) & 1] = 0xFFFFu;
             else *row = 0xFFFFFFFFu;
         }
@@ -602,7 +603,7 @@
     part[(static_cast<size_t>(split) * 2 + side) * Gp + g] = slot_pack(mn, mx);
 }
 
-__global__ __launch_bounds__(256) void k1_slot_keys(const uint32_t *__restrict__ part, int Gp, int G, uint32_t *__restrict__ gmm, uint32_t *__restrict__ key)
+__global__ __launch_bounds__(256) void k1_slot_keys(const uint32_t *__restrict__ part, int Gp, int G, int sides, uint32_t *__restrict__ gmm, uint32_t *__restrict__ key)
 {
     const int g = blockIdx.x * 256 + threadIdx.x;
     if (g >= G) return;
@@ -613,31 +614,68 @@
         r1 = slot_join(r1, part[(static_cast<size_t>(y) * 2 + 1) * Gp + g]);
     }
     gmm[g] = r0; gmm[Gp + g] = r1;
-    key[g] = slot_key(r0, r1);
-}
-
-__global__ __launch_bounds__(256) void k1_slot_rank(const uint32_t *__restrict__ key, int G, uint32_t *__restrict__ g2s)
-{
-    __shared__ uint64_t sk[kSlotRankSpan];
-    const int h0 = blockIdx.y * kSlotRankSpan;
-    for (int t = threadIdx.x; t < kSlotRankSpan; t += 256)
-        sk[t] = h0 + t < G ? slot_order_key(key[h0 + t], static_cast<uint32_t>(h0 + t)) : ~0ull;
+    if (sides == 2) { key[g] = slot_side_key(r0); key[Gp + g] = slot_side_key(r1); }
+    else key[g] = slot_key(r0, r1);
+}
+
+template <bool K32>
+__global__ __launch_bounds__(kSlotRankSpan / 2) void k1_slot_sort(const uint32_t *__restrict__ key, int G, int Gp, void *__restrict__ srt_)
+{
+    typedef typename std::conditional<K32, uint32_t, uint64_t>::type Key;
+    __shared__ Key sk[kSlotRankSpan];
+    key += static_cast<size_t>(blockIdx.y) * Gp;
+    Key *srt = static_cast<Key *>(srt_) + (static_cast<size_t>(blockIdx.y) * gridDim.x + blockIdx.x) * kSlotRankSpan;
+    const int h0 = blockIdx.x * kSlotRankSpan, t = threadIdx.x;
+    for (int e = t; e < kSlotRankSpan; e += kSlotRankSpan / 2) {
+        Key v = static_cast<Key>(~0ull);
+        if (h0 + e < G) {
+            if constexpr (K32) v = slot_order_key32(key[h0 + e], static_cast<uint32_t>(h0 + e));
+            else v = slot_order_key(key[h0 + e], static_cast<uint32_t>(h0 + e));
+        }
+        sk[e] = v;
+    }
+    for (int k = 2; k <= kSlotRankSpan; k <<= 1)
+        for (int j = k >> 1; j > 0; j >>= 1) {
+            __syncthreads();
+            const int l = ((t & ~(j - 1)) << 1) | (t & (j - 1)), r = l | j;
+            const Key x = sk[l], y = sk[r];
+            if ((x > y) == ((l & k) == 0)) { sk[l] = y; sk[r] = x; }
+        }
+    __syncthreads();
+    for (int e = t; e < kSlotRankSpan; e += kSlotRankSpan / 2) srt[e] = sk[e];
+}
+
+template <bool K32>
+__global__ __launch_bounds__(256) void k1_slot_rank(const uint32_t *__restrict__ key, const void *__restrict__ srt_, int G, int Gp, uint32_t *__restrict__ g2s)
+{
+    typedef typename std::conditional<K32, uint32_t, uint64_t>::type Key;
+    __shared__ Key sk[kSlotRankSpan];
+    key += static_cast<size_t>(blockIdx.z) * Gp; g2s += static_cast<size_t>(blockIdx.z) * Gp;
+    const Key *srt = static_cast<const Key *>(srt_) + (static_cast<size_t>(blockIdx.z) * gridDim.y + blockIdx.y) * kSlotRankSpan;
+    for (int t = threadIdx.x; t < kSlotRankSpan; t += 256) sk[t] = srt[t];
     __syncthreads();
     const int g = blockIdx.x * 256 + threadIdx.x;
     if (g >= G) return;
-    const uint64_t mine = slot_order_key(key[g], static_cast<uint32_t>(g));
+    Key mine;
+    if constexpr (K32) mine = slot_order_key32(key[g], static_cast<uint32_t>(g));
+    else mine = slot_order_key(key[g], static_cast<uint32_t>(g));
     uint32_t n = 0;
-#pragma unroll 8
-    for (int t = 0; t < kSlotRankSpan; ++t) n += sk[t] < mine ? 1u : 0u;
+#pragma unroll
+    for (int step = kSlotRankSpan / 2; step > 0; step >>= 1) n += sk[n + step - 1] < mine ? step : 0;
+    n += sk[n] < mine ? 1u : 0u;
     if (n) atomicAdd(&g2s[g], n);
 }
 
-__global__ __launch_bounds__(256) void k1_slot_invert(uint32_t *__restrict__ g2s, uint32_t *__restrict__ s2g, int G, int Gp)
+__global__ __launch_bounds__(256) void k1_slot_invert(uint32_t *__restrict__ g2s, uint32_t *__restrict__ s2g, int G, int Gp, int sides)
 {
     const int g = blockIdx.x * 256 + threadIdx.x;
     if (g >= Gp) return;
-    if (g < G) { const uint32_t k = g2s[g]; if (k < static_cast<uint32_t>(G)) s2g[k] = static_cast<uint32_t>(g); }
-    else { g2s[g] = static_cast<uint32_t>(g); s2g[g] = static_cast<uint32_t>(g); }
+    if (sides == 2) { g2s += static_cast<size_t>(blockIdx.y) * Gp; s2g += static_cast<size_t>(blockIdx.y) * Gp; }
+    uint32_t k = static_cast<uint32_t>(g), v = static_cast<uint32_t>(g);
+    if (g < G) { k = g2s[g]; if (k >= static_cast<uint32_t>(G)) return; }
+    else g2s[g] = v;
+    s2g[k] = v;
+    if (sides != 2) s2g[static_cast<size_t>(Gp) + k] = v;
 }
 
 __global__ __launch_bounds__(256) void k1_slot_ranges(const uint32_t *__restrict__ gmm, const uint32_t *__restrict__ s2g, int G, int Gp,
@@ -646,7 +684,7 @@
     static_assert(kSlotTile == kTileI && kSlotChunk == 64 * kRJ, "k1_slots.h carries its own copy of the item geometry");
     __shared__ uint32_t sm[8];
     const int k = blockIdx.x * 256 + threadIdx.x, side = blockIdx.y;
-    uint32_t r = k < G ? gmm[static_cast<size_t>(side) * Gp + s2g[k]] : slot_pack(kSlotNoMin, kSlotNoMax);
+    uint32_t r = k < G ? gmm[static_cast<size_t>(side) * Gp + s2g[static_cast<size_t>(side) * Gp + k]] : slot_pack(kSlotNoMin, kSlotNoMax);
 #pragma unroll
     for (int o = 1; o < 32; o <<= 1) r = slot_join(r, static_cast<uint32_t>(__shfl_xor(static_cast<int>(r), o)));
     if ((threadIdx.x & 31) == 0) { trng[static_cast<size_t>(side) * (Gp >> 5) + (k >> 5)] = r; sm[threadIdx.x >> 5] = r; }
@@ -657,10 +695,11 @@
     }
 }
 
-__global__ __launch_bounds__(256) void k1_slot_gather(const uint4 *__restrict__ P, const uint4 *__restrict__ AL, const uint32_t *__restrict__ s2g, int Gp,
+__global__ __launch_bounds__(256) void k1_slot_gather(const uint4 *__restrict__ P, const uint4 *__restrict__ AL, const uint32_t *__restrict__ s2g, int Gp, int cb, int ce,
                                                       uint4 *__restrict__ Ps, uint4 *__restrict__ ALs)
 {
     const int k = blockIdx.x * 256 + threadIdx.x, b = blockIdx.y;
+    if (b < cb || b >= ce) s2g += Gp;
     const uint32_t g = s2g[k];
 #pragma unroll
     for (int q = 0; q < 4; ++q) Ps[(static_cast<size_t>(b) * 4 + q) * Gp + k] = P[(static_cast<size_t>(b) * 4 + q) * Gp + g];
@@ -745,6 +784,38 @@
 #pragma unroll
         for (int q = 0; q < NQ; ++q)
             if (q < nq) rows[static_cast<size_t>(q) * Wp + wo] = u[q];
+    }
+}
+
+template <int R>
+__global__ __launch_bounds__(kUnslotThreadsMax) void k1_unslot_pair(uint32_t *__restrict__ table, const uint32_t *__restrict__ g2s, int G, int Wp)
+{
+    constexpr int NQ = 4 * R;
+    extern __shared__ uint32_t unslot_t[];
+    const int r0 = blockIdx.x * 2 * R, nr = min(2 * R, G - r0), side = blockIdx.y;
+    if (nr <= 0) return;
+    const int nq = nr * 2;
+    g2s += static_cast<size_t>(side) * 32 * Wp;
+    uint32_t *rows = table + static_cast<size_t>(r0) * kPlanes * Wp;
+    for (int w = threadIdx.x; w < Wp; w += blockDim.x) {
+        uint32_t m[NQ];
+#pragma unroll
+        for (int q = 0; q < NQ; ++q) m[q] = q < nq ? rows[unslot_pair_word(q, side, Wp, w)] : 0u;
+        unslot_in_word<R>(m, w, unslot_t);
+    }
+    __syncthreads();
+    for (int wo = threadIdx.x; wo < Wp; wo += blockDim.x) {
+        const uint4 *kq = reinterpret_cast<const uint4 *>(g2s) + static_cast<size_t>(wo) * 8;
+        uint32_t ks[32], u[NQ];
+#pragma unroll
+        for (int i = 0; i < 8; ++i) {
+            const uint4 k4 = kq[i];
+            ks[4 * i] = k4.x; ks[4 * i + 1] = k4.y; ks[4 * i + 2] = k4.z; ks[4 * i + 3] = k4.w;
+        }
+        unslot_out_word<R>(u, ks, wo, unslot_t, G, 32 * Wp);
+#pragma unroll
+        for (int q = 0; q < NQ; ++q)
+            if (q < nq) rows[unslot_pair_word(q, side, Wp, wo)] = u[q];
     }
 }
 
@@ -3785,15 +3856,16 @@
 }
 
 
-struct SlotMaps { uint32_t *gmm, *key, *g2s, *s2g, *trng, *crng; unsigned long long *count; };
-static size_t slot_maps_words(int Gp) { return static_cast<size_t>(Gp) * 5 + static_cast<size_t>(Gp) / 16 + static_cast<size_t>(Gp) / 128 + 2; }
+struct SlotMaps { uint32_t *gmm, *key, *g2s, *s2g, *trng, *crng; unsigned long long *count, *srt; };
+static size_t slot_maps_words(int Gp) { return static_cast<size_t>(Gp) * 8 + static_cast<size_t>(Gp) / 16 + static_cast<size_t>(Gp) / 128 + 2 + 4 * (static_cast<size_t>(Gp) + kSlotRankSpan); }
 static SlotMaps slot_maps(const reo_ctx *c)
 {
     SlotMaps m;
     const size_t Gp = static_cast<size_t>(c->Gp);
-    m.gmm = c->k1_slot_maps.p; m.key = m.gmm + 2 * Gp; m.g2s = m.key + Gp; m.s2g = m.g2s + Gp;
-    m.trng = m.s2g + Gp; m.crng = m.trng + Gp / 16;
+    m.gmm = c->k1_slot_maps.p; m.key = m.gmm + 2 * Gp; m.g2s = m.key + 2 * Gp; m.s2g = m.g2s + 2 * Gp;
+    m.trng = m.s2g + 2 * Gp; m.crng = m.trng + Gp / 16;
     m.count = reinterpret_cast<unsigned long long *>(m.crng + Gp / 128);
+    m.srt = m.count + 1;
     return m;
 }
 
@@ -3814,18 +3886,25 @@
     return REO_OK;
 }
 
-static int32_t k1_slots_front(reo_ctx *c, K1Args &a)
+static int32_t k1_slots_front(reo_ctx *c, K1Args &a, int sides)
 {
     const int G = a.G, Gp = a.Gp, nblk = c->goff32[2] / 32;
     const SlotMaps m = slot_maps(c);
-    const unsigned gb = static_cast<unsigned>((G + 255) / 256);
-    REO_HIP_CHECK(hipMemsetAsync(m.g2s, 0, static_cast<size_t>(Gp) * 2 * sizeof(uint32_t), c->stream));
+    const unsigned gb = static_cast<unsigned>((G + 255) / 256), zs = static_cast<unsigned>(sides);
+    REO_HIP_CHECK(hipMemsetAsync(m.g2s, 0, static_cast<size_t>(Gp) * 4 * sizeof(uint32_t), c->stream));
     k1_slot_part<<<dim3(gb, kSlotSplits, 2), 256, 0, c->stream>>>(c->t_pos16.p, Gp, G, a.cb * 32, a.nc, a.tb * 32, a.nt, c->k1_slot_part.p);
-    k1_slot_keys<<<gb, 256, 0, c->stream>>>(c->k1_slot_part.p, Gp, G, m.gmm, m.key);
-    k1_slot_rank<<<dim3(gb, static_cast<unsigned>((G + kSlotRankSpan - 1) / kSlotRankSpan)), 256, 0, c->stream>>>(m.key, G, m.g2s);
-    k1_slot_invert<<<static_cast<unsigned>(Gp / 256), 256, 0, c->stream>>>(m.g2s, m.s2g, G, Gp);
+    k1_slot_keys<<<gb, 256, 0, c->stream>>>(c->k1_slot_part.p, Gp, G, sides, m.gmm, m.key);
+    const unsigned spans = static_cast<unsigned>((G + kSlotRankSpan - 1) / kSlotRankSpan);
+    if (slot_order_key32_fits(G)) {
+        k1_slot_sort<true><<<dim3(spans, zs), kSlotRankSpan / 2, 0, c->stream>>>(m.key, G, Gp, m.srt);
+        k1_slot_rank<true><<<dim3(gb, spans, zs), 256, 0, c->stream>>>(m.key, m.srt, G, Gp, m.g2s);
+    } else {
+        k1_slot_sort<false><<<dim3(spans, zs), kSlotRankSpan / 2, 0, c->stream>>>(m.key, G, Gp, m.srt);
+        k1_slot_rank<false><<<dim3(gb, spans, zs), 256, 0, c->stream>>>(m.key, m.srt, G, Gp, m.g2s);
+    }
+    k1_slot_invert<<<dim3(static_cast<unsigned>(Gp / 256), zs), 256, 0, c->stream>>>(m.g2s, m.s2g, G, Gp, sides);
     k1_slot_ranges<<<dim3(static_cast<unsigned>(Gp / 256), 2), 256, 0, c->stream>>>(m.gmm, m.s2g, G, Gp, m.trng, m.crng);
-    k1_slot_gather<<<dim3(static_cast<unsigned>(Gp / 256), static_cast<unsigned>(nblk)), 256, 0, c->stream>>>(c->pos.p, c->lo.p, m.s2g, Gp, c->pos_s.p, c->lo_s.p);
+    k1_slot_gather<<<dim3(static_cast<unsigned>(Gp / 256), static_cast<unsigned>(nblk)), 256, 0, c->stream>>>(c->pos.p, c->lo.p, m.s2g, Gp, a.cb, a.ce, c->pos_s.p, c->lo_s.p);
     REO_HIP_CHECK(hipGetLastError());
     a.P = c->pos_s.p; a.AL = c->lo_s.p; a.AH = c->lo_s.p;
     a.s2g = m.s2g; a.trng = m.trng; a.crng = m.crng;
@@ -3837,7 +3916,7 @@
     return REO_OK;
 }
 
-static int32_t k1_slots_back(reo_ctx *c, const K1Args &a)
+static int32_t k1_slots_back(reo_ctx *c, const K1Args &a, int sides)
 {
     if (c->k1_unslot != 0) {
         int form = unslot_form(a.Gp);
@@ -3846,12 +3925,17 @@
         if (lds <= kUnslotLdsLimit) {
             auto go = [&](auto rtag) -> int32_t {
                 constexpr int R = decltype(rtag)::value;
-                const int bit = R == kUnslotWide ? 1 : 2;
+                const int bit = (R == kUnslotWide ? 1 : 2) << (sides == 2 ? 2 : 0);
+                const void *fn = sides == 2 ? reinterpret_cast<const void *>(k1_unslot_pair<R>) : reinterpret_cast<const void *>(k1_unslot_words<R>);
                 if (!(c->k1_unslot_attr & bit)) {
-                    REO_HIP_CHECK(hipFuncSetAttribute(reinterpret_cast<const void *>(k1_unslot_words<R>), hipFuncAttributeMaxDynamicSharedMemorySize, static_cast<int>(kUnslotLdsLimit)));
+                    REO_HIP_CHECK(hipFuncSetAttribute(fn, hipFuncAttributeMaxDynamicSharedMemorySize, static_cast<int>(kUnslotLdsLimit)));
                     c->k1_unslot_attr |= bit;
                 }
-                k1_unslot_words<R><<<static_cast<unsigned>((a.G + R - 1) / R), static_cast<unsigned>(unslot_threads(a.Wp)), lds, c->stream>>>(a.table, slot_maps(c).g2s, a.G, a.Wp);
+                const unsigned threads = static_cast<unsigned>(unslot_threads(a.Wp));
+                if (sides == 2)
+                    k1_unslot_pair<R><<<dim3(static_cast<unsigned>((a.G + 2 * R - 1) / (2 * R)), 2), threads, lds, c->stream>>>(a.table, slot_maps(c).g2s, a.G, a.Wp);
+                else
+                    k1_unslot_words<R><<<static_cast<unsigned>((a.G + R - 1) / R), threads, lds, c->stream>>>(a.table, slot_maps(c).g2s, a.G, a.Wp);
                 return REO_OK;
             };
             const int32_t rc = form == kUnslotWide ? go(std::integral_constant<int, kUnslotWide>{}) : go(std::integral_constant<int, kUnslotNarrow>{});
@@ -3861,6 +3945,7 @@
             return REO_OK;
         }
     }
+    if (sides != 1) { set_error("the bit form of the column un-permute: the common slot order only"); return REO_EINVAL; }
     c->last_k1_unslot = 1;
     const size_t row_bytes = static_cast<size_t>(a.Wp) * 16;
     auto go = [&](auto rtag) {
@@ -3914,7 +3999,7 @@
     if ((rc = upload_unit_map(c, units))) return rc;
     a.unit_map = c->unit_map.p;
     a.gate = gate;
-    if (!prepare) { c->last_k1_slots = 0; c->k1_slot_items = nullptr; c->k1_slot_items_n = 0; c->k1_slot_gp = 0; }
+    if (!prepare) { c->last_k1_slots = 0; c->last_k1_slot_sides = 0; c->k1_slot_items = nullptr; c->k1_slot_items_n = 0; c->k1_slot_gp = 0; }
     if ((range || prepare) && (sides != 1 && sides != 2)) { set_error("a range of sample blocks / a prepared launch: one side of the pair kernel"); return REO_EINVAL; }
     if (gate && (!pl.wave || pl.wide || pl.big)) { set_error("a gated launch of the pair kernel: wave form, at most 65535 genes and samples"); return REO_EINVAL; }
     c->x_pipelined = false;
@@ -3951,12 +4036,13 @@
     }
     if (a.stamps) k_time_mark<<<1, 64, 0, c->stream>>>(a.stamps + c->k1_items_n * 4);
     tic(c, 1);
-    if (pl.slots && (rc = k1_slots_front(c, a))) { toc(c); return rc; }
+    const int slot_sides = !pl.slots ? 0 : (c->k1_unslot == 0 ? 1 : slot_sides_wanted(a.ce - a.cb, a.te - a.tb, c->k1_slot_sides));
+    if (pl.slots && (rc = k1_slots_front(c, a, slot_sides))) { toc(c); return rc; }
     dispatch_pairs(c, a, pl);
-    if (pl.slots && (rc = k1_slots_back(c, a))) { toc(c); return rc; }
+    if (pl.slots && (rc = k1_slots_back(c, a, slot_sides))) { toc(c); return rc; }
     toc(c);
     if (pl.slots) {
-        c->last_k1_slots = 1;
+        c->last_k1_slots = 1; c->last_k1_slot_sides = slot_sides;
         c->k1_slot_items = a.items; c->k1_slot_items_n = c->k1_items_n; c->k1_slot_gp = a.Gp;
     }
     if (a.stamps) k_time_mark<<<1, 64, 0, c->stream>>>(a.stamps + c->k1_items_n * 4 + 1);
diff --git a/rankcompv3.jl_amd/csrc/reo_internal.h b/rankcompv3.jl_amd/csrc/reo_internal.h
--- a/rankcompv3.jl_amd/csrc/reo_internal.h
+++ b/rankcompv3.jl_amd/csrc/reo_internal.h
@@ -229,6 +229,8 @@
     int k1_slots = 1;
     int last_k1_slots = 0;
     int k1_unslot = -1;
+    int k1_slot_sides = 0;
+    int last_k1_slot_sides = 0;
     int last_k1_unslot = 0;
     int k1_unslot_attr = 0;
     const uint32_t *k1_slot_items = nullptr;
```

New measurement: 50980 billion (median of 6 runs). 4.3% higher.
